# Team766/ros_vision

Measured on NVIDIA B200. Metric: frames/s, higher is better.
Workload: dtype u8

## Files before the change

ros_vision_b200/csrc/kernels_blobs.cu:

```cuda
#include <cuda_runtime.h>
#include <math_constants.h>
#include <stdint.h>

#include <mutex>

#include "dev_types.h"
#include "kernels.h"

namespace b200tag {

static inline unsigned cdivu(unsigned a, unsigned b) { return (a + b - 1) / b; }
__host__ __device__ constexpr uint32_t next_pow2(uint32_t v) { uint32_t r = 1; while (r < v) r <<= 1; return r; }
constexpr uint32_t kMediumCap = 768;
constexpr uint32_t kSortCap = 4096;

__device__ __forceinline__ bool select_blob(const FrameParams &p, uint32_t count, uint32_t minx, uint32_t miny, uint32_t maxx,
                                            uint32_t maxy, int32_t gx, int32_t gy, long long dotsum) {
  if (count < p.min_cluster_pixels) return false;
  if (count > p.max_cluster_pixels) return false;
  if (static_cast<int>((maxx - minx) * (maxy - miny)) < p.min_tag_width) return false;
  const long long a = dotsum * 2 - static_cast<long long>(static_cast<int>(minx + maxx) * gx) -
                      static_cast<long long>(static_cast<int>(miny + maxy) * gy);
  const double d = static_cast<double>(a) * 0.5 - 0.05118 * static_cast<double>(gx) + 0.028581 * static_cast<double>(gy);
  const bool quad_reversed = static_cast<float>(d) < 0.0;
  if (!p.reversed_border && quad_reversed) return false;
  if (!p.normal_border && !quad_reversed) return false;
  return true;
}

template <int MIN_CTAS>
__global__ void __launch_bounds__(256, MIN_CTAS) k_select(FrameParams p) {
  __shared__ uint32_t s_warp[8][6];
  __shared__ unsigned long long s_base;
  __shared__ uint32_t s_pbase, s_mbase, s_lbase, s_hbase;
  const int frame = blockIdx.y;
  const size_t hoff = static_cast<size_t>(frame) * p.hash_cap;
  Counters *ctr = p.counters + frame;
  b200tag_blob *blobs = p.blobs + static_cast<size_t>(frame) * p.blob_cap;
  WorkItem *small_list = p.small_list + static_cast<size_t>(frame) * p.blob_cap;
  WorkItem *large_list = p.large_list + static_cast<size_t>(frame) * p.blob_cap;
  b200tag_blob *clusters = p.clusters ? p.clusters + static_cast<size_t>(frame) * p.cluster_cap : nullptr;
  const int lane = threadIdx.x & 31, warp = threadIdx.x >> 5;
  const uint32_t nocc = min(ctr->num_occupied, p.hash_cap);
  const uint32_t *occupied = p.occupied + hoff;
  const uint32_t nround = (nocc + blockDim.x - 1) / blockDim.x * blockDim.x;
  for (uint32_t oi = blockIdx.x * blockDim.x + threadIdx.x; oi < nround; oi += gridDim.x * blockDim.x) {
    const bool occ = oi < nocc;
    const uint32_t slot = occ ? occupied[oi] : 0u;
    const unsigned long long key = occ ? p.h_key[hoff + slot] : kEmptyKey;
    b200tag_blob rec;
    bool sel = false;
    if (occ) {
      rec.rep0 = static_cast<uint32_t>(key >> 32);
      rec.rep1 = static_cast<uint32_t>(key);
      rec.min_x = 0xffffffffu; rec.min_y = 0xffffffffu; rec.max_x = 0; rec.max_y = 0;
      rec.count = p.h_count[hoff + slot];
      rec.gx_sum = 0; rec.gy_sum = 0; rec.pxgx_plus_pygy_sum = 0;
      rec.slot = slot;
      rec.offset = 0;
      sel = rec.count >= p.min_cluster_pixels && rec.count <= p.max_cluster_pixels;
      rec.selected = 0;
      p.h_key[hoff + slot] = kEmptyKey;
      p.h_count[hoff + slot] = 0;
    }
    const bool small = sel && rec.count <= kSmallBlobPoints;
    const bool medium = sel && !small && rec.count <= kMediumCap;
    const bool huge = sel && rec.count > kSortCap;
    const uint32_t occ_mask = __ballot_sync(0xffffffffu, occ);
    const uint32_t sel_mask = __ballot_sync(0xffffffffu, sel);
    const uint32_t small_mask = __ballot_sync(0xffffffffu, small);
    const uint32_t medium_mask = __ballot_sync(0xffffffffu, medium);
    const uint32_t huge_mask = __ballot_sync(0xffffffffu, huge);
    uint32_t incl = sel ? rec.count : 0u;
#pragma unroll
    for (int o = 1; o < 32; o <<= 1) {
      const uint32_t t = __shfl_up_sync(0xffffffffu, incl, o);
      if (lane >= o) incl += t;
    }
    const uint32_t warp_pts = __shfl_sync(0xffffffffu, incl, 31);
    if (lane == 0) {
      s_warp[warp][0] = __popc(occ_mask);
      s_warp[warp][1] = __popc(sel_mask);
      s_warp[warp][2] = __popc(small_mask);
      s_warp[warp][3] = warp_pts;
      s_warp[warp][4] = __popc(medium_mask);
      s_warp[warp][5] = __popc(huge_mask);
    }
    __syncthreads();
    if (threadIdx.x == 0) {
      uint32_t t0 = 0, t1 = 0, t2 = 0, t3 = 0, t4 = 0, t5 = 0;
      for (int w = 0; w < 8; w++) {
        const uint32_t a0 = s_warp[w][0], a1 = s_warp[w][1], a2 = s_warp[w][2], a3 = s_warp[w][3], a4 = s_warp[w][4], a5 = s_warp[w][5];
        s_warp[w][0] = t0; s_warp[w][1] = t1; s_warp[w][2] = t2; s_warp[w][3] = t3; s_warp[w][4] = t4; s_warp[w][5] = t5;
        t0 += a0; t1 += a1; t2 += a2; t3 += a3; t4 += a4; t5 += a5;
      }
      unsigned long long base = 0;
      uint32_t pb = 0, mb = 0, lb = 0, hb = 0;
      if (t0) {
        const unsigned long long add = (static_cast<unsigned long long>(t0) << 40) | (static_cast<unsigned long long>(t1) << 20) | t2;
        base = atomicAdd(&ctr->alloc, add);
        if (t3) pb = atomicAdd(&ctr->num_seg_points, t3);
        if (t4) mb = atomicAdd(&ctr->num_medium, t4);
        if (t1 - t2 - t4 - t5) lb = atomicAdd(&ctr->num_large, t1 - t2 - t4 - t5);
        if (t5) hb = atomicAdd(&ctr->num_huge, t5);
      }
      s_base = base;
      s_pbase = pb;
      s_mbase = mb;
      s_lbase = lb;
      s_hbase = hb;
    }
    __syncthreads();
    const unsigned long long base = s_base;
    const uint32_t cbase = static_cast<uint32_t>(base >> 40) + s_warp[warp][0];
    const uint32_t bbase = static_cast<uint32_t>(base >> 20) & 0xfffffu;
    const uint32_t sbase = static_cast<uint32_t>(base) & 0xfffffu;
    uint32_t seg_off = 0xffffffffu;
    if (sel) {
      const uint32_t bw = s_warp[warp][1] + __popc(sel_mask & ((1u << lane) - 1u));
      const uint32_t sw = s_warp[warp][2] + __popc(small_mask & ((1u << lane) - 1u));
      const uint32_t mw = s_warp[warp][4] + __popc(medium_mask & ((1u << lane) - 1u));
      const uint32_t hw = s_warp[warp][5] + __popc(huge_mask & ((1u << lane) - 1u));
      const uint32_t cta_pos = medium ? s_mbase + mw
                             : (huge ? p.blob_cap - 1u - (s_hbase + hw) : p.blob_cap - 1u - (s_lbase + (bw - sw - mw - hw)));
      const uint32_t b = bbase + bw;
      const uint32_t off = s_pbase + s_warp[warp][3] + incl - rec.count;
      if (b < p.blob_cap && static_cast<uint64_t>(off) + rec.count <= p.point_cap) {
        rec.offset = off;
        blobs[b] = rec;
        seg_off = off;
        const WorkItem item{b, off, rec.count, 0u};
        if (small) small_list[sbase + sw] = item;
        else if (huge) small_list[cta_pos] = item;
        else large_list[cta_pos] = item;
      } else {
        atomicOr(&ctr->status, B200TAG_ST_BLOBS_OVERFLOW);
        const WorkItem none{0xffffffffu, 0u, 0u, 0u};
        if (small) {
          if (sbase + sw < p.blob_cap) small_list[sbase + sw] = none;
        } else if (cta_pos < p.blob_cap) {
          (huge ? small_list : large_list)[cta_pos] = none;
        }
      }
    }
    if (occ && clusters) {
      const uint32_t c = cbase + __popc(occ_mask & ((1u << lane) - 1u));
      if (c < p.cluster_cap) clusters[c] = rec;
      p.slot_cluster[hoff + slot] = c;
    }
    if (occ) p.slot_off[hoff + slot] = seg_off;
    __syncthreads();
  }
}

template <int U>
__global__ void __launch_bounds__(256) k_scatter(FrameParams p) {
  const int frame = blockIdx.y;
  const Counters *ctr = p.counters + frame;
  const uint32_t np = min(ctr->num_points, p.point_cap);
  const uint64_t *points = p.points + static_cast<size_t>(frame) * p.point_cap;
  const uint32_t *slot_off = p.slot_off + static_cast<size_t>(frame) * p.hash_cap;
  uint32_t *seg = p.seg_pts + static_cast<size_t>(frame) * p.point_cap;
  const uint32_t stride = gridDim.x * blockDim.x;
  for (uint32_t i = blockIdx.x * blockDim.x + threadIdx.x; i < np; i += U * stride) {
    uint64_t pt[U];
    uint32_t off[U];
#pragma unroll
    for (int u = 0; u < U; u++) {
      const uint32_t j = i + u * stride;
      pt[u] = (j < np && j >= i) ? __ldcs(points + j) : ~0ull;
    }
#pragma unroll
    for (int u = 0; u < U; u++) {
      const uint32_t slot = point_slot(pt[u]);
      off[u] = slot < p.hash_cap ? __ldg(slot_off + slot) : 0xffffffffu;
    }
#pragma unroll
    for (int u = 0; u < U; u++)
      if (off[u] != 0xffffffffu) seg[off[u] + point_rank(pt[u])] = point_seg(pt[u]);
  }
}

__global__ void __launch_bounds__(256) k_cluster_extents(FrameParams p) {
  const int frame = blockIdx.y;
  const Counters *ctr = p.counters + frame;
  const uint32_t np = min(ctr->num_points, p.point_cap);
  const uint64_t *points = p.points + static_cast<size_t>(frame) * p.point_cap;
  const uint32_t *slot_cluster = p.slot_cluster + static_cast<size_t>(frame) * p.hash_cap;
  b200tag_blob *clusters = p.clusters + static_cast<size_t>(frame) * p.cluster_cap;
  for (uint32_t i = blockIdx.x * blockDim.x + threadIdx.x; i < np; i += gridDim.x * blockDim.x) {
    const uint64_t pt = points[i];
    const uint32_t slot = point_slot(pt);
    if (slot >= p.hash_cap) continue;
    const uint32_t c = slot_cluster[slot];
    if (c >= p.cluster_cap) continue;
    const uint32_t sp = point_seg(pt);
    const int x = static_cast<int>(sp_x(sp)), y = static_cast<int>(sp_y(sp));
    const int d = static_cast<int>(sp_dir(sp));
    const int gx = sp_b2w(sp) ? dir_dx(d) : -dir_dx(d), gy = sp_b2w(sp) ? dir_dy(d) : -dir_dy(d);
    b200tag_blob *r = clusters + c;
    atomicMin(&r->min_x, static_cast<uint32_t>(x));
    atomicMax(&r->max_x, static_cast<uint32_t>(x));
    atomicMin(&r->min_y, static_cast<uint32_t>(y));
    atomicMax(&r->max_y, static_cast<uint32_t>(y));
    if (gx) atomicAdd(&r->gx_sum, gx);
    if (gy) atomicAdd(&r->gy_sum, gy);
    const int dot = x * gx + y * gy;
    if (dot) atomicAdd(reinterpret_cast<unsigned long long *>(&r->pxgx_plus_pygy_sum), static_cast<unsigned long long>(static_cast<long long>(dot)));
  }
}

__global__ void __launch_bounds__(256) k_cluster_finish(FrameParams p) {
  const int frame = blockIdx.y;
  const Counters *ctr = p.counters + frame;
  const uint32_t nc = min(alloc_clusters(ctr->alloc), p.cluster_cap);
  b200tag_blob *clusters = p.clusters + static_cast<size_t>(frame) * p.cluster_cap;
  for (uint32_t c = blockIdx.x * blockDim.x + threadIdx.x; c < nc; c += gridDim.x * blockDim.x) {
    b200tag_blob *r = clusters + c;
    r->selected = select_blob(p, r->count, r->min_x, r->min_y, r->max_x, r->max_y, r->gx_sum, r->gy_sum, r->pxgx_plus_pygy_sum);
  }
}

constexpr int kLargeThreads = 256;
constexpr int kSmallWarps = 4;

template <int GS>
__device__ __forceinline__ void gsync() {
  if constexpr (GS == 32) __syncwarp();
  else __syncthreads();
}

__device__ __forceinline__ void cmpxchg(unsigned long long *a, uint32_t i, uint32_t l) {
  const unsigned long long x = a[i], y = a[l];
  if (x > y) {
    a[i] = y;
    a[l] = x;
  }
}

template <int GS>
__device__ __noinline__ void bitonic_sort(unsigned long long *a, uint32_t cnt, uint32_t N, uint32_t gt) {
  const uint32_t half = N >> 1;
  for (uint32_t k = 2, lk = 1; k <= N; k <<= 1, lk++) {
    const uint32_t hk = k >> 1;
    for (uint32_t t = gt; t < half; t += GS) {
      const uint32_t blk = t >> (lk - 1), w = t & (hk - 1);
      const uint32_t i = (blk << lk) + w, l = (blk << lk) + k - 1 - w;
      if (l < cnt) cmpxchg(a, i, l);
    }
    if (GS > 32 && (k > 64 || (k == 2 ? false : (k >> 2) >= 64))) __syncthreads();
    else __syncwarp();
    for (uint32_t j = k >> 2; j > 0; j >>= 1) {
      for (uint32_t t = gt; t < half; t += GS) {
        const uint32_t i = ((t & ~(j - 1)) << 1) | (t & (j - 1)), l = i + j;
        if (l < cnt) cmpxchg(a, i, l);
      }
      const bool this_wide = j >= 64;
      const bool next_wide = (j > 1) ? ((j >> 1) >= 64) : ((k << 1) > 64);
      if (GS > 32 && (this_wide || next_wide)) __syncthreads();
      else __syncwarp();
    }
  }
  gsync<GS>();
}

struct Mom {
  long long Mx, My, W, Mxx, Myy, Mxy;
  int N;
};

struct LfStore {
  b200tag_lfp *aos;
  unsigned long long *m64;
  uint32_t *m32;
  uint32_t cap;
};
template <bool AOS>
__device__ __forceinline__ b200tag_lfp lf_load(const LfStore &L, uint32_t i) {
  if constexpr (AOS) return L.aos[i];
  b200tag_lfp r;
  r.Mxx = static_cast<long long>(L.m64[i]);
  r.Myy = static_cast<long long>(L.m64[L.cap + i]);
  r.Mxy = static_cast<long long>(L.m64[2 * L.cap + i]);
  r.Mx = L.m32[i];
  r.My = L.m32[L.cap + i];
  r.W = L.m32[2 * L.cap + i];
  return r;
}
template <bool AOS>
__device__ __forceinline__ void lf_store(const LfStore &L, uint32_t i, const b200tag_lfp &r) {
  if constexpr (AOS) {
    L.aos[i] = r;
    return;
  }
  L.m64[i] = static_cast<unsigned long long>(r.Mxx);
  L.m64[L.cap + i] = static_cast<unsigned long long>(r.Myy);
  L.m64[2 * L.cap + i] = static_cast<unsigned long long>(r.Mxy);
  L.m32[i] = static_cast<uint32_t>(r.Mx);
  L.m32[L.cap + i] = static_cast<uint32_t>(r.My);
  L.m32[2 * L.cap + i] = static_cast<uint32_t>(r.W);
}

template <bool AOS>
__device__ __forceinline__ Mom read_moments(const LfStore &lf, uint32_t cnt, uint32_t i0, uint32_t i1) {
  Mom m;
  if (i0 < i1) {
    m.N = static_cast<int>(i1 - i0 + 1);
    const b200tag_lfp a = lf_load<AOS>(lf, i1);
    m.Mx = a.Mx; m.My = a.My; m.Mxx = a.Mxx; m.Mxy = a.Mxy; m.Myy = a.Myy; m.W = a.W;
    if (i0 > 0) {
      const b200tag_lfp b = lf_load<AOS>(lf, i0 - 1);
      m.Mx -= b.Mx; m.My -= b.My; m.Mxx -= b.Mxx; m.Mxy -= b.Mxy; m.Myy -= b.Myy; m.W -= b.W;
    }
  } else {
    const b200tag_lfp b = lf_load<AOS>(lf, i0 - 1), z = lf_load<AOS>(lf, cnt - 1), a = lf_load<AOS>(lf, i1);
    m.Mx = z.Mx - b.Mx + a.Mx;
    m.My = z.My - b.My + a.My;
    m.Mxx = z.Mxx - b.Mxx + a.Mxx;
    m.Mxy = z.Mxy - b.Mxy + a.Mxy;
    m.Myy = z.Myy - b.Myy + a.Myy;
    m.W = z.W - b.W + a.W;
    m.N = static_cast<int>(cnt - i0 + i1 + 1);
  }
  return m;
}

__device__ __forceinline__ float eig_small_of(const Mom &m, float *hyp_out, long long *Cxx_o, long long *Cxy_o, long long *Cyy_o) {
  const long long Cxx = m.Mxx * m.W - m.Mx * m.Mx;
  const long long Cxy = m.Mxy * m.W - m.Mx * m.My;
  const long long Cyy = m.Myy * m.W - m.My * m.My;
  const float hyp = hypotf(static_cast<float>(Cxx - Cyy), static_cast<float>(2 * Cxy));
  const float eight_w2 = static_cast<float>(static_cast<double>(m.W * m.W) * 8.0);
  const float eig = (static_cast<float>(Cxx + Cyy) - hyp) / eight_w2;
  if (hyp_out) *hyp_out = hyp;
  if (Cxx_o) { *Cxx_o = Cxx; *Cxy_o = Cxy; *Cyy_o = Cyy; }
  return eig;
}

__device__ __forceinline__ void fit_line(const Mom &m, double *lp01, double *lp23, double *err, double *mse) {
  float hyp;
  long long Cxx, Cxy, Cyy;
  const float eig = eig_small_of(m, &hyp, &Cxx, &Cxy, &Cyy);
  if (lp01) {
    lp01[0] = static_cast<double>(static_cast<float>(m.Mx) / static_cast<float>(m.W * 2));
    lp01[1] = static_cast<double>(static_cast<float>(m.My) / static_cast<float>(m.W * 2));
  }
  if (lp23) {
    const float nx1 = static_cast<float>(Cxx - Cyy) - hyp;
    const float ny1 = static_cast<float>(2 * Cxy);
    const float M1 = nx1 * nx1 + ny1 * ny1;
    const float nx2 = static_cast<float>(2 * Cxy);
    const float ny2 = static_cast<float>(Cyy - Cxx) - hyp;
    const float M2 = nx2 * nx2 + ny2 * ny2;
    float nx, ny;
    if (M1 > M2) { nx = nx1; ny = ny1; } else { nx = nx2; ny = ny2; }
    const float len = hypotf(nx, ny);
    lp23[0] = static_cast<double>(nx / len);
    lp23[1] = static_cast<double>(ny / len);
  }
  *err = static_cast<double>(static_cast<float>(m.N) * eig);
  *mse = static_cast<double>(eig);
}

__device__ __forceinline__ int point_weight(const uint8_t *im, int w, int h, int ix, int iy) {
  int W = 1;
  if (ix > 0 && ix + 1 < w && iy > 0 && iy + 1 < h) {
    const int gx = static_cast<int>(__ldg(im + iy * w + ix + 1)) - static_cast<int>(__ldg(im + iy * w + ix - 1));
    const int gy = static_cast<int>(__ldg(im + (iy + 1) * w + ix)) - static_cast<int>(__ldg(im + (iy - 1) * w + ix));
    W = static_cast<int>(__fsqrt_rn(static_cast<float>(gx * gx + gy * gy)) + 1);
  }
  return W;
}

__device__ __forceinline__ uint32_t float_order(float f) {
  const uint32_t u = __float_as_uint(f + 0.0f);
  return (u & 0x80000000u) ? ~u : (u | 0x80000000u);
}

constexpr unsigned long long kNoKey = 0xFFFFFFFFFFFFFFFFull;
constexpr double kDblMax = 1.7976931348623157e308;

template <int WARPS>
struct BlobScratch {
  uint32_t peak_idx[kMaxPeaks];
  uint32_t red_u[WARPS > 1 ? WARPS : 1][4];
  int red_i[WARPS > 1 ? WARPS : 1][3];
  uint32_t npeaks;
  uint32_t nsel;
  uint32_t cur;
};

struct alignas(16) QuadScratch {
  double seg_err[kMaxPeaks][kMaxPeaks];
  double seg_nx[kMaxPeaks][kMaxPeaks], seg_ny[kMaxPeaks][kMaxPeaks];
  double lines[4][4];
  float corners[4][2];
  alignas(16) PeakTable t;
};

__device__ uint8_t d_combos[kNumCombos][4];

__global__ void k_init_combos() {
  int c = 0;
  for (int m0 = 0; m0 < kMaxPeaks - 3; m0++)
    for (int m1 = m0 + 1; m1 < kMaxPeaks - 2; m1++)
      for (int m2 = m1 + 1; m2 < kMaxPeaks - 1; m2++)
        for (int m3 = m2 + 1; m3 < kMaxPeaks; m3++) {
          d_combos[c][0] = m0; d_combos[c][1] = m1; d_combos[c][2] = m2; d_combos[c][3] = m3;
          c++;
        }
}

constexpr int kPeakRegs = 8;

template <int K>
__device__ __forceinline__ unsigned long long top_peaks_regs(const unsigned long long *peaks, uint32_t npk, int lane, uint32_t *nsel_out) {
  static_assert(K == 2 || K == 4 || K == 8, "sorting networks below");
  unsigned long long k[K];
#pragma unroll
  for (int j = 0; j < K; j++) {
    const uint32_t q = static_cast<uint32_t>(lane) + 32u * j;
    k[j] = q < npk ? peaks[q] : kNoKey;
  }
  constexpr int net2[1][2] = {{0, 1}};
  constexpr int net4[5][2] = {{0, 1}, {2, 3}, {0, 2}, {1, 3}, {1, 2}};
  constexpr int net8[19][2] = {{0, 1}, {2, 3}, {4, 5}, {6, 7}, {0, 2}, {1, 3}, {4, 6}, {5, 7}, {1, 2}, {5, 6},
                               {0, 4}, {3, 7}, {1, 5}, {2, 6}, {1, 4}, {3, 6}, {2, 4}, {3, 5}, {3, 4}};
  constexpr int ncmp = K == 2 ? 1 : (K == 4 ? 5 : 19);
#pragma unroll
  for (int c = 0; c < ncmp; c++) {
    const int i0 = K == 2 ? net2[c % 1][0] : (K == 4 ? net4[c % 5][0] : net8[c][0]);
    const int i1 = K == 2 ? net2[c % 1][1] : (K == 4 ? net4[c % 5][1] : net8[c][1]);
    const unsigned long long a = k[i0 % K], b2 = k[i1 % K];
    k[i0 % K] = a < b2 ? a : b2;
    k[i1 % K] = a < b2 ? b2 : a;
  }
  unsigned long long chosen = kNoKey;
  uint32_t nsel = 0;
#pragma unroll 1
  for (int round = 0; round < kMaxPeaks; round++) {
    const uint32_t hi = static_cast<uint32_t>(k[0] >> 32);
    const uint32_t mhi = __reduce_min_sync(0xffffffffu, hi);
    const uint32_t lo = (hi == mhi) ? static_cast<uint32_t>(k[0]) : 0xffffffffu;
    const uint32_t mlo = __reduce_min_sync(0xffffffffu, lo);
    const unsigned long long best = (static_cast<unsigned long long>(mhi) << 32) | mlo;
    if (best == kNoKey) break;
    nsel++;
    if (lane == round) chosen = best;
    if (k[0] == best) {
#pragma unroll
      for (int j = 0; j + 1 < K; j++) k[j] = k[j + 1];
      k[K - 1] = kNoKey;
    }
  }
  *nsel_out = nsel;
  return chosen;
}

__device__ __noinline__ uint32_t top_peaks_many(const unsigned long long *peaks, uint32_t npk, uint32_t *peak_idx, int lane) {
  unsigned long long last = 0;
  uint32_t nsel = 0;
#pragma unroll 1
  for (int round = 0; round < kMaxPeaks; round++) {
    unsigned long long best = kNoKey;
#pragma unroll 1
    for (uint32_t i = lane; i < npk; i += 32) {
      const unsigned long long key = peaks[i];
      if ((round == 0 || key > last) && key < best) best = key;
    }
    {
      const uint32_t hi = static_cast<uint32_t>(best >> 32);
      const uint32_t mhi = __reduce_min_sync(0xffffffffu, hi);
      const uint32_t lo = (hi == mhi) ? static_cast<uint32_t>(best) : 0xffffffffu;
      const uint32_t mlo = __reduce_min_sync(0xffffffffu, lo);
      best = (static_cast<unsigned long long>(mhi) << 32) | mlo;
    }
    if (best == kNoKey) break;
    last = best;
    nsel++;
    if (lane == 0) {
      const uint32_t v2 = static_cast<uint32_t>(best & 0xffffffffu);
      int q = static_cast<int>(nsel) - 2;
      while (q >= 0 && peak_idx[q] > v2) { peak_idx[q + 1] = peak_idx[q]; q--; }
      peak_idx[q + 1] = v2;
    }
    __syncwarp();
  }
  return nsel;
}

struct BlobWork {
  unsigned long long *keys;
  LfStore lf;
  float *errs;
  double *filt;
  unsigned long long *peaks;
  bool keys_in_place;
  uint32_t *hist;
  uint32_t hist_cap;
  uint32_t *tmp;
};

constexpr uint32_t kMaxBucketLoad = 24;

template <int GS, bool AOS, bool KEEP>
__device__ __forceinline__ void fit_one_blob(const FrameParams &p, int frame, Counters *ctr, uint32_t b, uint32_t cnt, uint32_t off,
                                             b200tag_blob *blob_rec, const BlobWork &wk, BlobScratch<GS / 32> &S, long long *scan, uint32_t gt) {
  const size_t n = static_cast<size_t>(p.w) * p.h;
  const uint8_t *quad = p.quad + frame * n;
  const size_t pbase = static_cast<size_t>(frame) * p.point_cap + off;
  const int lane = threadIdx.x & 31;
  const bool first_warp = gt < 32;

  uint32_t *raw = reinterpret_cast<uint32_t *>(wk.errs);
  {
    const uint32_t N = 1u << (32 - __clz(static_cast<int>(cnt - 1)));
    const uint32_t B = min(N, wk.hist_cap);
    for (uint32_t i = gt; i < B; i += GS) wk.hist[i] = 0;
    if (gt == 0) S.npeaks = 0;
    const uint32_t *sp = p.seg_pts + pbase;
    uint32_t mnx = 0xffffffffu, mxx = 0, mny = 0xffffffffu, mxy = 0;
    int sgx = 0, sgy = 0, sdot = 0;
    for (uint32_t i = gt; i < cnt; i += GS) {
      const uint32_t v = __ldcg(sp + i);
      raw[i] = v;
      const uint32_t x = sp_x(v), y = sp_y(v);
      const int d = static_cast<int>(sp_dir(v));
      const int gx = sp_b2w(v) ? dir_dx(d) : -dir_dx(d), gy = sp_b2w(v) ? dir_dy(d) : -dir_dy(d);
      mnx = min(mnx, x); mxx = max(mxx, x); mny = min(mny, y); mxy = max(mxy, y);
      sgx += gx; sgy += gy;
      sdot += static_cast<int>(x) * gx + static_cast<int>(y) * gy;
    }
    mnx = __reduce_min_sync(0xffffffffu, mnx); mxx = __reduce_max_sync(0xffffffffu, mxx);
    mny = __reduce_min_sync(0xffffffffu, mny); mxy = __reduce_max_sync(0xffffffffu, mxy);
    sgx = __reduce_add_sync(0xffffffffu, sgx); sgy = __reduce_add_sync(0xffffffffu, sgy);
    sdot = __reduce_add_sync(0xffffffffu, sdot);
    if constexpr (GS > 32) {
      const int wi = gt >> 5;
      if (lane == 0) {
        S.red_u[wi][0] = mnx; S.red_u[wi][1] = mxx; S.red_u[wi][2] = mny; S.red_u[wi][3] = mxy;
        S.red_i[wi][0] = sgx; S.red_i[wi][1] = sgy; S.red_i[wi][2] = sdot;
      }
      __syncthreads();
      mnx = 0xffffffffu; mxx = 0; mny = 0xffffffffu; mxy = 0; sgx = 0; sgy = 0; sdot = 0;
#pragma unroll
      for (int w = 0; w < GS / 32; w++) {
        mnx = min(mnx, S.red_u[w][0]); mxx = max(mxx, S.red_u[w][1]); mny = min(mny, S.red_u[w][2]); mxy = max(mxy, S.red_u[w][3]);
        sgx += S.red_i[w][0]; sgy += S.red_i[w][1]; sdot += S.red_i[w][2];
      }
    }
    const bool sel = select_blob(p, cnt, mnx, mny, mxx, mxy, sgx, sgy, static_cast<long long>(sdot));
    if (gt == 0) {
      blob_rec->min_x = mnx; blob_rec->min_y = mny; blob_rec->max_x = mxx; blob_rec->max_y = mxy;
      blob_rec->gx_sum = sgx; blob_rec->gy_sum = sgy; blob_rec->pxgx_plus_pygy_sum = sdot;
      blob_rec->selected = sel;
      if (sel) {
        atomicAdd(&ctr->num_selected_blobs, 1u);
        atomicAdd(&ctr->num_selected_points, cnt);
      }
    }
    if (!sel) return;
    if constexpr (GS == 32) __syncwarp();
    const double cx = static_cast<double>(static_cast<float>(static_cast<int>(mnx + mxx)) * 0.5f) + 0.05118;
    const double cy = static_cast<double>(static_cast<float>(static_cast<int>(mny + mxy)) * 0.5f) + -0.028581;

    const uint32_t bk_shift = 26u - (31u - static_cast<uint32_t>(__clz(static_cast<int>(B))));
    uint32_t *th_tmp = wk.tmp, *rk_tmp = wk.tmp + cnt;
#pragma unroll 1
    for (uint32_t i = gt; i < cnt; i += GS) {
      const uint32_t v = raw[i];
      const float fy = static_cast<float>(static_cast<double>(sp_y(v)) - cy);
      const float fx = static_cast<float>(static_cast<double>(sp_x(v)) - cx);
      const float theta = static_cast<float>((static_cast<double>(atan2f(fy, fx)) + 3.14159265358979323846) * 8e6);
      long long ti = llrintf(theta);
      if (ti < 0) ti = 0;
      const uint32_t th = static_cast<uint32_t>(ti & 0xfffffff);
      const uint32_t bk = (th >> bk_shift);
      th_tmp[i] = th;
      rk_tmp[i] = atomicAdd(&wk.hist[bk], 1u);
    }
    gsync<GS>();
    const uint32_t per = B / GS;
    uint32_t sum = 0, mx = 0;
    for (uint32_t j = 0; j < per; j++) {
      const uint32_t c = wk.hist[gt * per + j];
      sum += c;
      mx = max(mx, c);
    }
    uint32_t incl = sum;
#pragma unroll
    for (int o = 1; o < 32; o <<= 1) {
      const uint32_t t = __shfl_up_sync(0xffffffffu, incl, o);
      if (lane >= o) incl += t;
    }
    mx = __reduce_max_sync(0xffffffffu, mx);
    if constexpr (GS > 32) {
      const int wi = gt >> 5;
      if (lane == 31) S.red_u[wi][0] = incl;
      if (lane == 0) S.red_u[wi][1] = mx;
      __syncthreads();
      uint32_t before = 0;
      mx = 0;
#pragma unroll
      for (int w = 0; w < GS / 32; w++) {
        if (w < wi) before += S.red_u[w][0];
        mx = max(mx, S.red_u[w][1]);
      }
      incl += before;
    }
    const bool bucketed = mx <= kMaxBucketLoad && !(p.test_flags & B200TAG_TEST_BITONIC_SORT);
    if (bucketed) {
      uint32_t ex = incl - sum;
      for (uint32_t j = 0; j < per; j++) {
        const uint32_t c = wk.hist[gt * per + j];
        wk.hist[gt * per + j] = ex;
        ex += c;
      }
      gsync<GS>();
      for (uint32_t i = gt; i < cnt; i += GS) {
        const uint32_t v = raw[i], th = th_tmp[i];
        const uint32_t bk = (th >> bk_shift);
        wk.keys[wk.hist[bk] + rk_tmp[i]] = pack_sort_key(th, sp_dir(v), sp_by(v), sp_bx(v));
      }
      gsync<GS>();
      constexpr uint32_t kRankPer = 6;
      if (cnt <= kRankPer * GS) {
        unsigned long long kreg[kRankPer];
        uint32_t preg[kRankPer];
#pragma unroll
        for (uint32_t j = 0; j < kRankPer; j++) {
          const uint32_t q = gt + j * GS;
          kreg[j] = 0;
          preg[j] = 0xffffffffu;
          if (q < cnt) {
            const unsigned long long key = wk.keys[q];
            const uint32_t bk = (key_theta(key) >> bk_shift);
            const uint32_t lo = wk.hist[bk], hi = (bk + 1 < B) ? wk.hist[bk + 1] : cnt;
            uint32_t pos = lo;
#pragma unroll 1
            for (uint32_t i = lo; i < hi; i++) pos += wk.keys[i] < key;
            kreg[j] = key;
            preg[j] = pos;
          }
        }
        gsync<GS>();
#pragma unroll
        for (uint32_t j = 0; j < kRankPer; j++)
          if (preg[j] != 0xffffffffu) wk.keys[preg[j]] = kreg[j];
      } else {
        for (uint32_t j = 0; j < per; j++) {
          const uint32_t bk = gt * per + j;
          const uint32_t lo = wk.hist[bk], hi = (bk + 1 < B) ? wk.hist[bk + 1] : cnt;
          for (uint32_t i = lo + 1; i < hi; i++) {
            const unsigned long long key = wk.keys[i];
            uint32_t q = i;
            while (q > lo && wk.keys[q - 1] > key) {
              wk.keys[q] = wk.keys[q - 1];
              q--;
            }
            wk.keys[q] = key;
          }
        }
      }
      gsync<GS>();
    } else {
      for (uint32_t i = gt; i < cnt; i += GS) {
        const uint32_t v = raw[i];
        wk.keys[i] = pack_sort_key(th_tmp[i], sp_dir(v), sp_by(v), sp_bx(v));
      }
      gsync<GS>();
      bitonic_sort<GS>(wk.keys, cnt, N, gt);
    }
  }
  if (KEEP && !wk.keys_in_place) {
    uint64_t *out = p.seg_keys + pbase;
#pragma unroll 1
    for (uint32_t i = gt; i < cnt; i += GS) out[i] = wk.keys[i];
  }

  int *wbuf = reinterpret_cast<int *>(wk.errs);
  if constexpr (!AOS) {
    {
      const int wi = static_cast<int>(gt >> 5);
      const uint32_t L = ((cnt + GS - 1) / GS) | 1u;
      const uint32_t c_lo = min(cnt, gt * L), c_hi = min(cnt, c_lo + L);
      unsigned long long t_Mxx = 0, t_Myy = 0, t_Mxy = 0;
      uint32_t t_Mx = 0, t_My = 0, t_W = 0;
  #pragma unroll 2
      for (uint32_t i = c_lo; i < c_hi; i++) {
        const unsigned long long k = wk.keys[i];
        const uint32_t d = key_dir(k);
        const uint32_t ix2 = 2 * key_bx(k) + dir_dx(d) + 1, iy2 = 2 * key_by(k) + dir_dy(d) + 1;
        const uint32_t W = static_cast<uint32_t>(point_weight(quad, p.w, p.h, static_cast<int>(ix2 / 2), static_cast<int>(iy2 / 2)));
        wbuf[i] = static_cast<int>(W);
        const uint32_t wx = W * ix2, wy = W * iy2;
        t_Mx += wx; t_My += wy; t_W += W;
        t_Mxx += static_cast<unsigned long long>(wx) * ix2;
        t_Mxy += static_cast<unsigned long long>(wx) * iy2;
        t_Myy += static_cast<unsigned long long>(wy) * iy2;
      }
      unsigned long long s_Mxx = t_Mxx, s_Myy = t_Myy, s_Mxy = t_Mxy, s_Mx = t_Mx, s_My = t_My, s_W = t_W;
  #pragma unroll
      for (int o = 1; o < 32; o <<= 1) {
        const unsigned long long u_Mxx = __shfl_up_sync(0xffffffffu, s_Mxx, o), u_Myy = __shfl_up_sync(0xffffffffu, s_Myy, o);
        const unsigned long long u_Mxy = __shfl_up_sync(0xffffffffu, s_Mxy, o);
        const uint32_t u_Mx = __shfl_up_sync(0xffffffffu, static_cast<uint32_t>(s_Mx), o), u_My = __shfl_up_sync(0xffffffffu, static_cast<uint32_t>(s_My), o);
        const uint32_t u_W = __shfl_up_sync(0xffffffffu, static_cast<uint32_t>(s_W), o);
        if (lane >= o) { s_Mx += u_Mx; s_My += u_My; s_W += u_W; s_Mxx += u_Mxx; s_Myy += u_Myy; s_Mxy += u_Mxy; }
      }
      unsigned long long c_Mxx = s_Mxx - t_Mxx, c_Myy = s_Myy - t_Myy, c_Mxy = s_Mxy - t_Mxy;
      unsigned long long c_Mx = s_Mx - t_Mx, c_My = s_My - t_My, c_W = s_W - t_W;
      if constexpr (GS > 32) {
        unsigned long long *tot = reinterpret_cast<unsigned long long *>(scan);
        if (lane == 31) {
          tot[wi * 6 + 0] = s_Mxx; tot[wi * 6 + 1] = s_Myy; tot[wi * 6 + 2] = s_Mxy;
          tot[wi * 6 + 3] = s_Mx;  tot[wi * 6 + 4] = s_My;  tot[wi * 6 + 5] = s_W;
        }
        __syncthreads();
        for (int w = 0; w < wi; w++) {
          c_Mxx += tot[w * 6 + 0]; c_Myy += tot[w * 6 + 1]; c_Mxy += tot[w * 6 + 2];
          c_Mx += tot[w * 6 + 3];  c_My += tot[w * 6 + 4];  c_W += tot[w * 6 + 5];
        }
      }
  #pragma unroll 2
      for (uint32_t i = c_lo; i < c_hi; i++) {
        const unsigned long long k = wk.keys[i];
        const uint32_t d = key_dir(k);
        const uint32_t ix2 = 2 * key_bx(k) + dir_dx(d) + 1, iy2 = 2 * key_by(k) + dir_dy(d) + 1;
        const uint32_t W = static_cast<uint32_t>(wbuf[i]);
        const uint32_t wx = W * ix2, wy = W * iy2;
        c_Mx += wx; c_My += wy; c_W += W;
        c_Mxx += static_cast<unsigned long long>(wx) * ix2;
        c_Mxy += static_cast<unsigned long long>(wx) * iy2;
        c_Myy += static_cast<unsigned long long>(wy) * iy2;
        b200tag_lfp o;
        o.Mxx = static_cast<long long>(c_Mxx); o.Myy = static_cast<long long>(c_Myy); o.Mxy = static_cast<long long>(c_Mxy);
        o.Mx = static_cast<long long>(c_Mx); o.My = static_cast<long long>(c_My); o.W = static_cast<long long>(c_W);
        lf_store<AOS>(wk.lf, i, o);
      }
    }
  } else {
  #pragma unroll 2
    for (uint32_t i = gt; i < cnt; i += GS) {
      const unsigned long long k = wk.keys[i];
      const uint32_t d = key_dir(k);
      const int ix2 = static_cast<int>(2 * key_bx(k)) + dir_dx(d) + 1, iy2 = static_cast<int>(2 * key_by(k)) + dir_dy(d) + 1;
      wbuf[i] = point_weight(quad, p.w, p.h, ix2 / 2, iy2 / 2);
    }
    gsync<GS>();
    {
      constexpr int kWarps = GS / 32;
      const int wi = static_cast<int>(gt >> 5);
      const uint32_t per_warp = ((cnt + kWarps - 1) / kWarps + 31u) & ~31u;
      const uint32_t w_lo = min(cnt, wi * per_warp), w_hi = min(cnt, w_lo + per_warp);
      unsigned long long c_Mxx = 0, c_Myy = 0, c_Mxy = 0, c_Mx = 0, c_My = 0, c_W = 0;
      if constexpr (GS > 32) {
        unsigned long long t_Mxx = 0, t_Myy = 0, t_Mxy = 0;
        uint32_t t_Mx = 0, t_My = 0, t_W = 0;
        for (uint32_t i = w_lo + lane; i < w_hi; i += 32) {
          const unsigned long long k = wk.keys[i];
          const uint32_t d = key_dir(k);
          const uint32_t ix2 = 2 * key_bx(k) + dir_dx(d) + 1, iy2 = 2 * key_by(k) + dir_dy(d) + 1;
          const uint32_t W = static_cast<uint32_t>(wbuf[i]);
          const uint32_t wx = W * ix2, wy = W * iy2;
          t_Mx += wx; t_My += wy; t_W += W;
          t_Mxx += static_cast<unsigned long long>(wx) * ix2;
          t_Mxy += static_cast<unsigned long long>(wx) * iy2;
          t_Myy += static_cast<unsigned long long>(wy) * iy2;
        }
        unsigned long long r_Mx = t_Mx, r_My = t_My, r_W = t_W;
  #pragma unroll
        for (int o = 16; o > 0; o >>= 1) {
          t_Mxx += __shfl_xor_sync(0xffffffffu, t_Mxx, o);
          t_Myy += __shfl_xor_sync(0xffffffffu, t_Myy, o);
          t_Mxy += __shfl_xor_sync(0xffffffffu, t_Mxy, o);
          r_Mx += __shfl_xor_sync(0xffffffffu, r_Mx, o);
          r_My += __shfl_xor_sync(0xffffffffu, r_My, o);
          r_W += __shfl_xor_sync(0xffffffffu, r_W, o);
        }
        unsigned long long *tot = reinterpret_cast<unsigned long long *>(scan);
        if (lane == 0) {
          tot[wi * 6 + 0] = t_Mxx; tot[wi * 6 + 1] = t_Myy; tot[wi * 6 + 2] = t_Mxy;
          tot[wi * 6 + 3] = r_Mx;  tot[wi * 6 + 4] = r_My;  tot[wi * 6 + 5] = r_W;
        }
        __syncthreads();
        for (int w = 0; w < wi; w++) {
          c_Mxx += tot[w * 6 + 0]; c_Myy += tot[w * 6 + 1]; c_Mxy += tot[w * 6 + 2];
          c_Mx += tot[w * 6 + 3];  c_My += tot[w * 6 + 4];  c_W += tot[w * 6 + 5];
        }
      }
  #pragma unroll 1
      for (uint32_t base = w_lo; base < w_hi; base += 32) {
        const uint32_t i = base + lane;
        uint32_t s_Mx = 0, s_My = 0, s_W = 0;
        unsigned long long s_Mxx = 0, s_Myy = 0, s_Mxy = 0;
        if (i < w_hi) {
          const unsigned long long k = wk.keys[i];
          const uint32_t d = key_dir(k);
          const uint32_t ix2 = 2 * key_bx(k) + dir_dx(d) + 1, iy2 = 2 * key_by(k) + dir_dy(d) + 1;
          const uint32_t W = static_cast<uint32_t>(wbuf[i]);
          const uint32_t wx = W * ix2, wy = W * iy2;
          s_Mx = wx; s_My = wy; s_W = W;
          s_Mxx = static_cast<unsigned long long>(wx) * ix2;
          s_Mxy = static_cast<unsigned long long>(wx) * iy2;
          s_Myy = static_cast<unsigned long long>(wy) * iy2;
        }
  #pragma unroll
        for (int o = 1; o < 32; o <<= 1) {
          const uint32_t u_Mx = __shfl_up_sync(0xffffffffu, s_Mx, o), u_My = __shfl_up_sync(0xffffffffu, s_My, o);
          const uint32_t u_W = __shfl_up_sync(0xffffffffu, s_W, o);
          const unsigned long long u_Mxx = __shfl_up_sync(0xffffffffu, s_Mxx, o), u_Myy = __shfl_up_sync(0xffffffffu, s_Myy, o);
          const unsigned long long u_Mxy = __shfl_up_sync(0xffffffffu, s_Mxy, o);
          if (lane >= o) { s_Mx += u_Mx; s_My += u_My; s_W += u_W; s_Mxx += u_Mxx; s_Myy += u_Myy; s_Mxy += u_Mxy; }
        }
        if (i < w_hi) {
          b200tag_lfp o;
          o.Mxx = static_cast<long long>(c_Mxx + s_Mxx); o.Myy = static_cast<long long>(c_Myy + s_Myy);
          o.Mxy = static_cast<long long>(c_Mxy + s_Mxy);
          o.Mx = static_cast<long long>(c_Mx + s_Mx); o.My = static_cast<long long>(c_My + s_My); o.W = static_cast<long long>(c_W + s_W);
          lf_store<AOS>(wk.lf, i, o);
        }
        c_Mxx += __shfl_sync(0xffffffffu, s_Mxx, 31); c_Myy += __shfl_sync(0xffffffffu, s_Myy, 31);
        c_Mxy += __shfl_sync(0xffffffffu, s_Mxy, 31);
        c_Mx += __shfl_sync(0xffffffffu, s_Mx, 31); c_My += __shfl_sync(0xffffffffu, s_My, 31); c_W += __shfl_sync(0xffffffffu, s_W, 31);
      }
    }
  }
  gsync<GS>();
  if (KEEP && !AOS) {
    b200tag_lfp *out = p.lfp + pbase;
#pragma unroll 1
    for (uint32_t i = gt; i < cnt; i += GS) out[i] = lf_load<AOS>(wk.lf, i);
  }

  const uint32_t ksz = min(20u, cnt / 12u);
#pragma unroll 1
  for (uint32_t i = gt; i < cnt; i += GS) {
    uint32_t i0 = i + cnt - ksz, i1 = i + ksz;
    if (i0 >= cnt) i0 -= cnt;
    if (i1 >= cnt) i1 -= cnt;
    const Mom m = read_moments<AOS>(wk.lf, cnt, i0, i1);
    const float eig = eig_small_of(m, nullptr, nullptr, nullptr, nullptr);
    wk.errs[i] = static_cast<float>(m.N) * eig;
  }
  gsync<GS>();
  if (KEEP && wk.errs != p.errs + pbase) {
    float *out = p.errs + pbase;
#pragma unroll 1
    for (uint32_t i = gt; i < cnt; i += GS) out[i] = wk.errs[i];
  }
#pragma unroll 1
  for (uint32_t i = gt; i < cnt; i += GS) {
    const float kf[7] = {0.01110899634659290314f, 0.13533528149127960205f, 0.60653066635131835938f, 1.0f,
                         0.60653066635131835938f, 0.13533528149127960205f, 0.01110899634659290314f};
    double acc = 0.0;
    uint32_t q = i + cnt - 3;
    if (q >= cnt) q -= cnt;
#pragma unroll
    for (int j = 0; j < 7; j++) {
      const double e = static_cast<double>(wk.errs[q]);
      acc += e * static_cast<double>(kf[j]);
      if (++q == cnt) q = 0;
    }
    wk.filt[i] = acc;
  }
  gsync<GS>();
  if (KEEP && wk.filt != p.filt + pbase) {
    double *out = p.filt + pbase;
#pragma unroll 1
    for (uint32_t i = gt; i < cnt; i += GS) out[i] = wk.filt[i];
  }

#pragma unroll 1
  for (uint32_t i = gt; i < cnt; i += GS) {
    const double m = wk.filt[i];
    const double bv = wk.filt[i == 0 ? cnt - 1 : i - 1], av = wk.filt[i + 1 == cnt ? 0 : i + 1];
    if (m > bv && m > av) {
      const uint32_t at = atomicAdd(&S.npeaks, 1u);
      wk.peaks[at] = (static_cast<unsigned long long>(float_order(static_cast<float>(-m))) << 32) | i;
    }
  }
  gsync<GS>();
  const uint32_t npk = S.npeaks;
  if (npk == 0) return;

  uint32_t fq_slot = 0;
  if (first_warp) {
    if (lane == 0) fq_slot = atomicAdd(&ctr->num_fit_quads, 1u);
    uint32_t nsel = 0;
    if (npk <= 32) {
      unsigned long long v = lane < static_cast<int>(npk) ? wk.peaks[lane] : kNoKey;
#pragma unroll
      for (int k = 2; k <= 32; k <<= 1) {
#pragma unroll
        for (int j = k >> 1; j > 0; j >>= 1) {
          const unsigned long long other = __shfl_xor_sync(0xffffffffu, v, j);
          const bool take_min = ((lane & k) == 0) == ((lane & j) == 0);
          v = (take_min == (other < v)) ? other : v;
        }
      }
      nsel = min(npk, static_cast<uint32_t>(kMaxPeaks));
      const uint32_t my_idx = static_cast<uint32_t>(v & 0xffffffffu);
      uint32_t rank = 0;
#pragma unroll
      for (int m = 0; m < kMaxPeaks; m++) {
        const uint32_t o = __shfl_sync(0xffffffffu, my_idx, m);
        rank += (m < static_cast<int>(nsel)) && (o < my_idx);
      }
      if (lane < static_cast<int>(nsel)) S.peak_idx[rank] = my_idx;
    } else if (npk <= 32 * kPeakRegs) {
      const unsigned long long chosen = npk <= 64    ? top_peaks_regs<2>(wk.peaks, npk, lane, &nsel)
                                        : npk <= 128 ? top_peaks_regs<4>(wk.peaks, npk, lane, &nsel)
                                                     : top_peaks_regs<8>(wk.peaks, npk, lane, &nsel);
      const uint32_t my_idx = static_cast<uint32_t>(chosen & 0xffffffffu);
      uint32_t rank = 0;
#pragma unroll
      for (int m = 0; m < kMaxPeaks; m++) {
        const uint32_t o = __shfl_sync(0xffffffffu, my_idx, m);
        rank += (m < static_cast<int>(nsel)) && (o < my_idx);
      }
      if (lane < static_cast<int>(nsel)) S.peak_idx[rank] = my_idx;
    } else {
      nsel = top_peaks_many(wk.peaks, npk, S.peak_idx, lane);
    }
    if (lane == 0) S.nsel = nsel;
    __syncwarp();
  }

  if (first_warp) {
    const uint32_t nm = S.nsel;
    const uint32_t fq = __shfl_sync(0xffffffffu, fq_slot, 0);
    if (fq < p.blob_cap) {
      PeakTable *t = p.peak_tables + static_cast<size_t>(frame) * p.blob_cap + fq;
      if (lane == 0) {
        t->blob = b; t->cnt = cnt; t->nsel = nm; t->npk = npk; t->rep0 = blob_rec->rep0; t->rep1 = blob_rec->rep1;
        t->last = lf_load<AOS>(wk.lf, cnt - 1);
      }
      if (lane < static_cast<int>(nm)) {
        const uint32_t i = S.peak_idx[lane];
        t->idx[lane] = i;
        t->at[lane] = lf_load<AOS>(wk.lf, i);
        b200tag_lfp z;
        z.Mxx = 0; z.Myy = 0; z.Mxy = 0; z.Mx = 0; z.My = 0; z.W = 0;
        t->before[lane] = i > 0 ? lf_load<AOS>(wk.lf, i - 1) : z;
      }
    }
  }
}

__device__ __forceinline__ Mom table_moments(const PeakTable &T, int a, int c) {
  const uint32_t i0 = T.idx[a], i1 = T.idx[c];
  const b200tag_lfp hi = T.at[c], lo = T.before[a];
  Mom m;
  if (i0 < i1) {
    m.N = static_cast<int>(i1 - i0 + 1);
    m.Mx = hi.Mx; m.My = hi.My; m.Mxx = hi.Mxx; m.Mxy = hi.Mxy; m.Myy = hi.Myy; m.W = hi.W;
    if (i0 > 0) { m.Mx -= lo.Mx; m.My -= lo.My; m.Mxx -= lo.Mxx; m.Mxy -= lo.Mxy; m.Myy -= lo.Myy; m.W -= lo.W; }
  } else {
    const b200tag_lfp z = T.last;
    m.Mx = z.Mx - lo.Mx + hi.Mx;
    m.My = z.My - lo.My + hi.My;
    m.Mxx = z.Mxx - lo.Mxx + hi.Mxx;
    m.Mxy = z.Mxy - lo.Mxy + hi.Mxy;
    m.Myy = z.Myy - lo.Myy + hi.Myy;
    m.W = z.W - lo.W + hi.W;
    m.N = static_cast<int>(T.cnt - i0 + i1 + 1);
  }
  return m;
}

constexpr int kQuadWarps = 4;

__global__ void __launch_bounds__(kQuadWarps * 32, 8) k_quads(FrameParams p) {
  __shared__ QuadScratch s_q[kQuadWarps];
  const int frame = blockIdx.y;
  const int lane = threadIdx.x & 31;
  QuadScratch &S = s_q[threadIdx.x >> 5];
  Counters *ctr = p.counters + frame;
  const uint32_t nfq = min(ctr->num_fit_quads, p.blob_cap);
  const PeakTable *tables = p.peak_tables + static_cast<size_t>(frame) * p.blob_cap;
  for (uint32_t fq = blockIdx.x * kQuadWarps + (threadIdx.x >> 5); fq < nfq; fq += gridDim.x * kQuadWarps) {
    __syncwarp();
    {
      constexpr uint32_t kPieces = sizeof(PeakTable) / 16, kPer = (kPieces + 31) / 32;
      const uint4 *src = reinterpret_cast<const uint4 *>(tables + fq);
      uint4 *dst = reinterpret_cast<uint4 *>(&S.t);
      uint4 v[kPer];
#pragma unroll
      for (uint32_t k = 0; k < kPer; k++)
        if (lane + 32 * k < kPieces) v[k] = __ldcg(src + lane + 32 * k);
#pragma unroll
      for (uint32_t k = 0; k < kPer; k++)
        if (lane + 32 * k < kPieces) dst[lane + 32 * k] = v[k];
    }
    __syncwarp();
    const PeakTable &T = S.t;
    const uint32_t b = T.blob, cnt = T.cnt, npk = T.npk;

  const int nm = static_cast<int>(T.nsel);
  const double max_mse = static_cast<double>(p.max_line_fit_mse);
  const uint32_t inv_nm1 = nm > 1 ? 65535u / static_cast<uint32_t>(nm - 1) + 1u : 0u;
  for (int t = lane; t < nm * (nm - 1); t += 32) {
    const int a = static_cast<int>((static_cast<uint32_t>(t) * inv_nm1) >> 16);
    int c = t - a * (nm - 1);
    c += c >= a;
    const Mom mo = table_moments(T, a, c);
    double err, mse, nrm[2] = {0.0, 0.0};
    fit_line(mo, nullptr, a < c ? nrm : nullptr, &err, &mse);
    S.seg_err[a][c] = (mse > max_mse) ? kDblMax : err;
    S.seg_nx[a][c] = nrm[0];
    S.seg_ny[a][c] = nrm[1];
  }
  __syncwarp();

  {
    const double max_dot = static_cast<double>(p.cos_critical_rad);
    double my_err = kDblMax;
    int my_rank = kNumCombos;
    for (int c = lane; c < kNumCombos; c += 32) {
      const uchar4 cm = *reinterpret_cast<const uchar4 *>(d_combos[c]);
      const int m0 = cm.x, m1 = cm.y, m2 = cm.z, m3 = cm.w;
      if (m3 >= nm) continue;
      const double e01 = S.seg_err[m0][m1];
      if (e01 == kDblMax) continue;
      const double e12 = S.seg_err[m1][m2];
      if (e12 == kDblMax) continue;
      const double dot = S.seg_nx[m0][m1] * S.seg_nx[m1][m2] + S.seg_ny[m0][m1] * S.seg_ny[m1][m2];
      if (fabs(dot) > max_dot) continue;
      const double e23 = S.seg_err[m2][m3];
      if (e23 == kDblMax) continue;
      const double e30 = S.seg_err[m3][m0];
      if (e30 == kDblMax) continue;
      const double tot = e01 + e12 + e23 + e30;
      if (tot < my_err) { my_err = tot; my_rank = c; }
    }
#pragma unroll
    for (int o = 16; o > 0; o >>= 1) {
      const double oe = __shfl_xor_sync(0xffffffffu, my_err, o);
      const int orank = __shfl_xor_sync(0xffffffffu, my_rank, o);
      if (oe < my_err || (oe == my_err && orank < my_rank)) { my_err = oe; my_rank = orank; }
    }

    const double best = my_err;
    const int bi = my_rank < kNumCombos ? my_rank : 0;
    const bool valid = best < static_cast<double>(p.max_line_fit_mse * static_cast<float>(cnt));
    b200tag_fit_quad *fqo = (fq < p.blob_cap) ? (p.fit_quads + static_cast<size_t>(frame) * p.blob_cap + fq) : nullptr;
    if (lane == 0 && fqo) {
      fqo->blob_index = b;
      fqo->valid = valid;
      fqo->num_peaks = static_cast<int32_t>(npk);
      fqo->err = best;
    }
    if (lane < 4) {
      uint32_t i0 = 0;
      Mom mo;
      if (valid) {
        i0 = T.idx[d_combos[bi][lane]];
        mo = table_moments(T, d_combos[bi][lane], d_combos[bi][(lane + 1) & 3]);
        double err, mse;
        fit_line(mo, S.lines[lane], S.lines[lane] + 2, &err, &mse);
      }
      if (fqo) {
        fqo->indices[lane] = i0;
        b200tag_moments mm = b200tag_moments{0, 0, 0, 0, 0, 0, 0, 0};
        if (valid) { mm.Mx = mo.Mx; mm.My = mo.My; mm.W = mo.W; mm.Mxx = mo.Mxx; mm.Myy = mo.Myy; mm.Mxy = mo.Mxy; mm.N = mo.N; }
        fqo->moments[lane] = mm;
      }
    }
    __syncwarp();
    if (valid) {
      bool bad = false;
      if (lane < 4) {
        const int i = lane, nx = (lane + 1) & 3;
        const double A00 = S.lines[i][3], A01 = -S.lines[nx][3];
        const double A10 = -S.lines[i][2], A11 = S.lines[nx][2];
        const double B0 = -S.lines[i][0] + S.lines[nx][0];
        const double B1 = -S.lines[i][1] + S.lines[nx][1];
        const double det = A00 * A11 - A10 * A01;
        const double W00 = A11 / det, W01 = -A01 / det;
        if (fabs(det) < 0.001) bad = true;
        const double L0 = W00 * B0 + W01 * B1;
        S.corners[i][0] = static_cast<float>(S.lines[i][0] + L0 * A00);
        S.corners[i][1] = static_cast<float>(S.lines[i][1] + L0 * A10);
      }
      bad = __any_sync(0xffffffffu, bad);
      __syncwarp();
      float elen = 0;
      if (lane < 6) {
        const int a = (0x032210 >> (4 * lane)) & 0xf, c = (0x203021 >> (4 * lane)) & 0xf;
        elen = hypotf(S.corners[c][0] - S.corners[a][0], S.corners[c][1] - S.corners[a][1]);
      }
      float elens[6];
#pragma unroll
      for (int i = 0; i < 6; i++) elens[i] = __shfl_sync(0xffffffffu, elen, i);
      if (lane == 0 && !bad) {
        float cr[4][2];
        for (int j = 0; j < 4; j++) { cr[j][0] = S.corners[j][0]; cr[j][1] = S.corners[j][1]; }
        {
          float area = 0;
          float pp;
          pp = (elens[0] + elens[1] + elens[2]) / 2;
          area += sqrtf(pp * (pp - elens[0]) * (pp - elens[1]) * (pp - elens[2]));
          pp = (elens[3] + elens[4] + elens[5]) / 2;
          area += sqrtf(pp * (pp - elens[3]) * (pp - elens[4]) * (pp - elens[5]));
          if (static_cast<double>(area) < 0.95 * p.min_tag_width * p.min_tag_width) bad = true;
        }
        if (!bad) {
          for (int i = 0; i < 4; i++) {
            const int i0 = i, i1 = (i + 1) & 3, i2 = (i + 2) & 3;
            const float dx1 = cr[i1][0] - cr[i0][0], dy1 = cr[i1][1] - cr[i0][1];
            const float dx2 = cr[i2][0] - cr[i1][0], dy2 = cr[i2][1] - cr[i1][1];
            const float cos_dtheta = (dx1 * dx2 + dy1 * dy2) / sqrtf((dx1 * dx1 + dy1 * dy1) * (dx2 * dx2 + dy2 * dy2));
            if (fabsf(cos_dtheta) > p.cos_critical_rad || dx1 * dy2 < dy1 * dx2) { bad = true; break; }
          }
        }
        if (!bad) {
          const float f = static_cast<float>(p.f);
          if (f > 1) {
            for (int j = 0; j < 4; j++) {
              cr[j][0] = (cr[j][0] - 0.5f) * f + 0.5f;
              cr[j][1] = (cr[j][1] - 0.5f) * f + 0.5f;
            }
          }
          const uint32_t qi = atomicAdd(&ctr->num_quads, 1u);
          if (qi < p.quad_cap) {
            b200tag_quad &q = (p.quads + static_cast<size_t>(frame) * p.quad_cap)[qi];
            for (int j = 0; j < 4; j++) { q.corners[j][0] = cr[j][0]; q.corners[j][1] = cr[j][1]; }
            q.reversed_border = p.reversed_border && !p.normal_border;
            q.blob_index = b;
            q.rep0 = T.rep0;
            q.rep1 = T.rep1;
          } else {
            atomicOr(&ctr->status, B200TAG_ST_QUADS_OVERFLOW);
          }
        }
      }
    }
  }
  }
}

struct SmallWarpShared {
  unsigned long long keys[kSmallBlobPoints];
  unsigned long long lf64[3 * kSmallBlobPoints];
  uint32_t lf32[3 * kSmallBlobPoints];
  alignas(16) float errs[kSmallBlobPoints];
  BlobScratch<1> scratch;
};

template <bool KEEP>
__global__ void __launch_bounds__(kSmallWarps * 32, 6) k_fit_small(FrameParams p) {
  extern __shared__ __align__(16) unsigned char smem_raw[];
  SmallWarpShared &S = reinterpret_cast<SmallWarpShared *>(smem_raw)[threadIdx.x >> 5];
  const int frame = blockIdx.y;
  const int lane = threadIdx.x & 31;
  Counters *ctr = p.counters + frame;
  b200tag_blob *blobs = p.blobs + static_cast<size_t>(frame) * p.blob_cap;
  const WorkItem *list = p.small_list + static_cast<size_t>(frame) * p.blob_cap;
  const uint32_t nlist = min(alloc_small(ctr->alloc), p.blob_cap);
  BlobWork wk;
  wk.keys = S.keys;
  wk.lf.aos = nullptr; wk.lf.m64 = S.lf64; wk.lf.m32 = S.lf32; wk.lf.cap = kSmallBlobPoints;
  wk.errs = S.errs;
  wk.filt = reinterpret_cast<double *>(S.keys);
  wk.peaks = reinterpret_cast<unsigned long long *>(S.errs);
  wk.keys_in_place = false;
  wk.hist = reinterpret_cast<uint32_t *>(S.lf64);
  wk.hist_cap = next_pow2(kSmallBlobPoints);
  wk.tmp = wk.hist + next_pow2(kSmallBlobPoints);
  uint32_t nxt = 0;
  if (lane == 0) nxt = atomicAdd(&ctr->next_small, 1u);
  while (true) {
    __syncwarp();
    const uint32_t li = __shfl_sync(0xffffffffu, nxt, 0);
    if (li >= nlist) break;
    if (lane == 0) nxt = atomicAdd(&ctr->next_small, 1u);
    const WorkItem item = list[li];
    const uint32_t b = item.blob, off = item.offset, cnt = item.count;
    if (b >= p.blob_cap) continue;
    if (cnt > kSmallBlobPoints) continue;
    fit_one_blob<32, false, KEEP>(p, frame, ctr, b, cnt, off, blobs + b, wk, S.scratch, nullptr, lane);
  }
}

template <int THREADS, uint32_t KEY_CAP, uint32_t LF_CAP>
struct CtaShared {
  static constexpr bool kHasB = KEY_CAP > LF_CAP;
  static constexpr uint32_t kScanWords = kHasB ? (KEY_CAP / 2 > 6 * THREADS ? KEY_CAP / 2 : 6 * THREADS) : 0;
  static constexpr size_t kBytesA = static_cast<size_t>(LF_CAP) * 48;
  static constexpr size_t kBytesB = kHasB ? static_cast<size_t>(KEY_CAP) * 12 + static_cast<size_t>(kScanWords) * 8 : 0;
  alignas(16) unsigned char buf[kBytesA > kBytesB ? kBytesA : kBytesB];
  long long tot[6 * (THREADS / 32)];
  BlobScratch<THREADS / 32> scratch;

  __device__ unsigned long long *a_keys() { return reinterpret_cast<unsigned long long *>(buf); }
  __device__ unsigned long long *a_lf64() { return reinterpret_cast<unsigned long long *>(buf) + LF_CAP; }
  __device__ uint32_t *a_lf32() { return reinterpret_cast<uint32_t *>(buf + static_cast<size_t>(LF_CAP) * 32); }
  __device__ float *a_errs() { return reinterpret_cast<float *>(buf + static_cast<size_t>(LF_CAP) * 44); }
  __device__ unsigned long long *b_keys() { return reinterpret_cast<unsigned long long *>(buf); }
  __device__ float *b_errs() { return reinterpret_cast<float *>(buf + static_cast<size_t>(KEY_CAP) * 8); }
  __device__ long long *b_scan() { return reinterpret_cast<long long *>(buf + static_cast<size_t>(KEY_CAP) * 12); }
};
static_assert(kMediumCap % 4 == 0 && kSortCap % 4 == 0, "16-byte alignment of the carved arrays");

template <int THREADS, uint32_t KEY_CAP, uint32_t LF_CAP, uint32_t MIN_CNT, uint32_t MAX_CNT, int MIN_CTAS, bool KEEP>
__global__ void __launch_bounds__(THREADS, MIN_CTAS) k_fit_cta(FrameParams p, int tier) {
  using Shared = CtaShared<THREADS, KEY_CAP, LF_CAP>;
  extern __shared__ __align__(16) unsigned char smem_raw[];
  Shared &S = *reinterpret_cast<Shared *>(smem_raw);
  const int frame = blockIdx.y;
  const int tid = threadIdx.x;
  Counters *ctr = p.counters + frame;
  b200tag_blob *blobs = p.blobs + static_cast<size_t>(frame) * p.blob_cap;
  const WorkItem *list = (tier == 2 ? p.small_list : p.large_list) + static_cast<size_t>(frame) * p.blob_cap;
  const uint32_t nlist = min(tier == 0 ? ctr->num_medium : (tier == 1 ? ctr->num_large : ctr->num_huge), p.blob_cap);
  constexpr uint32_t kScanHist = (KEY_CAP / 2 > 6 * THREADS) ? KEY_CAP : ((6u * THREADS * 2u >= 2048u) ? 2048u : 1024u);
  uint32_t *next = tier == 0 ? &ctr->next_medium : (tier == 1 ? &ctr->next_large : &ctr->next_huge);
  uint32_t nxt = 0;
  if (tid == 0) nxt = atomicAdd(next, 1u);
  while (true) {
    __syncthreads();
    if (tid == 0) S.scratch.cur = nxt;
    __syncthreads();
    const uint32_t li = S.scratch.cur;
    if (li >= nlist) break;
    if (tid == 0) nxt = atomicAdd(next, 1u);
    const WorkItem item = list[tier == 0 ? li : p.blob_cap - 1u - li];
    const uint32_t b = item.blob, blob_off = item.offset, blob_cnt = item.count;
    if (b >= p.blob_cap) continue;
    if (blob_cnt < MIN_CNT || blob_cnt > MAX_CNT) continue;
    const size_t pbase = static_cast<size_t>(frame) * p.point_cap + blob_off;
    BlobWork wk;
    constexpr bool kHasSmemLf = LF_CAP > 0;
    constexpr bool kHasGlobalLf = MAX_CNT > LF_CAP;
    constexpr bool kHasInPlace = MAX_CNT > KEY_CAP;
    const bool lf32_ok = LF_CAP <= 1452 || !kHasGlobalLf ||
                         static_cast<uint64_t>(blob_cnt) * 361u * (2u * static_cast<uint32_t>(max(p.w, p.h)) + 1u) < (1ull << 32);
    if (kHasSmemLf && blob_cnt <= LF_CAP && lf32_ok) {
      wk.keys = S.a_keys(); wk.errs = S.a_errs();
      wk.lf.aos = nullptr; wk.lf.m64 = S.a_lf64(); wk.lf.m32 = S.a_lf32(); wk.lf.cap = LF_CAP;
      wk.filt = reinterpret_cast<double *>(S.a_keys());
      wk.peaks = reinterpret_cast<unsigned long long *>(S.a_errs());
      wk.keys_in_place = false;
      wk.hist = reinterpret_cast<uint32_t *>(S.a_lf64()); wk.hist_cap = next_pow2(LF_CAP > 0 ? LF_CAP : 1); wk.tmp = wk.hist + next_pow2(LF_CAP > 0 ? LF_CAP : 1);
      fit_one_blob<THREADS, false, KEEP>(p, frame, ctr, b, blob_cnt, blob_off, blobs + b, wk, S.scratch, S.tot, tid);
    } else if (kHasGlobalLf && KEY_CAP > LF_CAP && blob_cnt <= KEY_CAP) {
      wk.keys = S.b_keys(); wk.errs = S.b_errs();
      wk.lf.aos = p.lfp + pbase; wk.lf.m64 = nullptr; wk.lf.m32 = nullptr; wk.lf.cap = 0;
      wk.filt = reinterpret_cast<double *>(S.b_keys());
      wk.peaks = reinterpret_cast<unsigned long long *>(S.b_errs());
      wk.keys_in_place = false;
      wk.hist = reinterpret_cast<uint32_t *>(S.b_scan()); wk.hist_cap = kScanHist; wk.tmp = reinterpret_cast<uint32_t *>(p.lfp + pbase);
      fit_one_blob<THREADS, true, KEEP>(p, frame, ctr, b, blob_cnt, blob_off, blobs + b, wk, S.scratch, S.b_scan(), tid);
    } else if (kHasInPlace) {
      wk.keys = reinterpret_cast<unsigned long long *>(p.seg_keys + pbase);
      wk.lf.aos = p.lfp + pbase; wk.lf.m64 = nullptr; wk.lf.m32 = nullptr; wk.lf.cap = 0;
      wk.errs = p.errs + pbase; wk.filt = p.filt + pbase;
      wk.peaks = reinterpret_cast<unsigned long long *>(p.peak_ws + static_cast<size_t>(frame) * (p.point_cap / 2 + 1) + blob_off / 2);
      wk.keys_in_place = true;
      wk.hist = reinterpret_cast<uint32_t *>(S.b_scan()); wk.hist_cap = kScanHist; wk.tmp = reinterpret_cast<uint32_t *>(p.lfp + pbase);
      fit_one_blob<THREADS, true, KEEP>(p, frame, ctr, b, blob_cnt, blob_off, blobs + b, wk, S.scratch, S.b_scan(), tid);
    }
  }
}

using MediumShared = CtaShared<128, kMediumCap, kMediumCap>;
constexpr uint32_t kLargeLfCap = 1536;
using LargeShared = CtaShared<kLargeThreads, kSortCap, kLargeLfCap>;
static_assert(sizeof(LargeShared) <= 76800 - 1024, "three CTAs of the large tier per SM");
static_assert(sizeof(MediumShared) <= 37888, "shared memory of the medium tier");
#define K_FIT_MEDIUM(KEEP) k_fit_cta<128, kMediumCap, kMediumCap, kSmallBlobPoints + 1, kMediumCap, 6, KEEP>
#define K_FIT_LARGE(KEEP) k_fit_cta<kLargeThreads, kSortCap, kLargeLfCap, kMediumCap + 1, kSortCap, 3, KEEP>
constexpr int kHugeThreads = 512;
constexpr uint32_t kHugeCap = 8192;
using HugeShared = CtaShared<kHugeThreads, kHugeCap, 0>;
#define K_FIT_HUGE(KEEP) k_fit_cta<kHugeThreads, kHugeCap, 0, kSortCap + 1, 0xffffffffu, (KEEP) ? 1 : 2, KEEP>
using Large512Shared = CtaShared<kHugeThreads, kSortCap, kSortCap>;
#define K_FIT_LARGE512(KEEP) k_fit_cta<kHugeThreads, kSortCap, kSortCap, kMediumCap + 1, kSortCap, 1, KEEP>
static_assert(sizeof(Large512Shared) <= 227 * 1024, "shared memory of the low-latency large tier");
constexpr int kLowLatencyFrames = 4;

void launch_blobs_init(cudaStream_t s) {
  static bool dev_ready[64] = {false};
  static std::mutex mu;
  std::lock_guard<std::mutex> lock(mu);
  int dev = 0;
  cudaGetDevice(&dev);
  if (dev >= 0 && dev < 64 && !dev_ready[dev]) {
    cudaFuncSetAttribute(k_fit_small<false>, cudaFuncAttributeMaxDynamicSharedMemorySize, static_cast<int>(sizeof(SmallWarpShared) * kSmallWarps));
    cudaFuncSetAttribute(k_fit_small<true>, cudaFuncAttributeMaxDynamicSharedMemorySize, static_cast<int>(sizeof(SmallWarpShared) * kSmallWarps));
    cudaFuncSetAttribute(K_FIT_MEDIUM(false), cudaFuncAttributeMaxDynamicSharedMemorySize, static_cast<int>(sizeof(MediumShared)));
    cudaFuncSetAttribute(K_FIT_MEDIUM(true), cudaFuncAttributeMaxDynamicSharedMemorySize, static_cast<int>(sizeof(MediumShared)));
    cudaFuncSetAttribute(K_FIT_LARGE(false), cudaFuncAttributeMaxDynamicSharedMemorySize, static_cast<int>(sizeof(LargeShared)));
    cudaFuncSetAttribute(K_FIT_LARGE(true), cudaFuncAttributeMaxDynamicSharedMemorySize, static_cast<int>(sizeof(LargeShared)));
    cudaFuncSetAttribute(K_FIT_HUGE(false), cudaFuncAttributeMaxDynamicSharedMemorySize, static_cast<int>(sizeof(HugeShared)));
    cudaFuncSetAttribute(K_FIT_HUGE(true), cudaFuncAttributeMaxDynamicSharedMemorySize, static_cast<int>(sizeof(HugeShared)));
    cudaFuncSetAttribute(K_FIT_LARGE512(false), cudaFuncAttributeMaxDynamicSharedMemorySize, static_cast<int>(sizeof(Large512Shared)));
    cudaFuncSetAttribute(K_FIT_LARGE512(true), cudaFuncAttributeMaxDynamicSharedMemorySize, static_cast<int>(sizeof(Large512Shared)));
    k_init_combos<<<1, 1, 0, s>>>();
    dev_ready[dev] = true;
  }
}

int launch_blobs(const FrameParams &p, int frames, cudaStream_t s, KernelTimer *kt, const SideStreams *side) {
  if (kt) kt->begin("select", s);
  if (exp_flags() & 64) k_select<1><<<dim3(max(1u, min(16u, cdivu(148u * 4u, frames))), frames), 256, 0, s>>>(p);
  else k_select<8><<<dim3(max(1u, min(16u, 148u * 8u / static_cast<unsigned>(frames))), frames), 256, 0, s>>>(p);
  if (kt) kt->end(s);
  if (kt) kt->begin("scatter", s);
  if (exp_flags() & 1) k_scatter<1><<<dim3(max(8u, min(592u, cdivu(4736u, frames))), frames), 256, 0, s>>>(p);
  else if (exp_flags() & 32) k_scatter<8><<<dim3(max(8u, min(592u, cdivu(4736u, frames))), frames), 256, 0, s>>>(p);
  else k_scatter<4><<<dim3(max(8u, min(592u, cdivu(4736u, frames))), frames), 256, 0, s>>>(p);
  if (kt) kt->end(s);
  int launches = 6;
  if (p.clusters) {
    k_cluster_extents<<<dim3(max(8u, min(592u, cdivu(4736u, frames))), frames), 256, 0, s>>>(p);
    k_cluster_finish<<<dim3(16, frames), 256, 0, s>>>(p);
    launches += 2;
  }
  const bool fork = side && side->s[0] && side->s[1] && side->s[2];
  cudaStream_t s_large = fork ? side->s[0] : s, s_medium = fork ? side->s[1] : s, s_huge = fork ? side->s[2] : s;
  if (fork) {
    cudaEventRecord(side->fork, s);
    cudaStreamWaitEvent(s_large, side->fork, 0);
    cudaStreamWaitEvent(s_medium, side->fork, 0);
    cudaStreamWaitEvent(s_huge, side->fork, 0);
  }
  if (kt) kt->begin("fit_huge", s);
  {
    const dim3 g(max(1u, min(148u, cdivu(592u, frames))), frames);
    if (p.keep_stages) K_FIT_HUGE(true)<<<g, kHugeThreads, sizeof(HugeShared), s_huge>>>(p, 2);
    else K_FIT_HUGE(false)<<<g, kHugeThreads, sizeof(HugeShared), s_huge>>>(p, 2);
  }
  if (kt) kt->end(s);
  if (kt) kt->begin("fit_large", s);
  const bool lf32_ok = static_cast<uint64_t>(kSortCap) * 361u * (2u * static_cast<uint32_t>(max(p.w, p.h)) + 1u) < (1ull << 32);
  if (frames <= kLowLatencyFrames && lf32_ok) {
    const dim3 g(max(1u, min(148u, cdivu(592u, frames))), frames);
    if (p.keep_stages) K_FIT_LARGE512(true)<<<g, kHugeThreads, sizeof(Large512Shared), s_large>>>(p, 1);
    else K_FIT_LARGE512(false)<<<g, kHugeThreads, sizeof(Large512Shared), s_large>>>(p, 1);
  } else {
    const dim3 g(max(3u, min(444u, cdivu(1776u, frames))), frames);
    if (p.keep_stages) K_FIT_LARGE(true)<<<g, kLargeThreads, sizeof(LargeShared), s_large>>>(p, 1);
    else K_FIT_LARGE(false)<<<g, kLargeThreads, sizeof(LargeShared), s_large>>>(p, 1);
  }
  if (kt) kt->end(s);
  if (kt) kt->begin("fit_medium", s);
  {
    const dim3 g(max(4u, min(740u, cdivu(2960u, frames))), frames);
    if (p.keep_stages) K_FIT_MEDIUM(true)<<<g, 128, sizeof(MediumShared), s_medium>>>(p, 0);
    else K_FIT_MEDIUM(false)<<<g, 128, sizeof(MediumShared), s_medium>>>(p, 0);
  }
  if (kt) kt->end(s);
  if (kt) kt->begin("fit_small", s);
  {
    const dim3 g(max(4u, min(740u, cdivu(2960u, frames))), frames);
    if (p.keep_stages) k_fit_small<true><<<g, kSmallWarps * 32, sizeof(SmallWarpShared) * kSmallWarps, s>>>(p);
    else k_fit_small<false><<<g, kSmallWarps * 32, sizeof(SmallWarpShared) * kSmallWarps, s>>>(p);
  }
  if (kt) kt->end(s);
  if (fork) {
    cudaEventRecord(side->join[0], s_large);
    cudaEventRecord(side->join[1], s_medium);
    cudaEventRecord(side->join[2], s_huge);
    cudaStreamWaitEvent(s, side->join[0], 0);
    cudaStreamWaitEvent(s, side->join[1], 0);
    cudaStreamWaitEvent(s, side->join[2], 0);
  }
  if (kt) kt->begin("quads", s);
  k_quads<<<dim3(max(2u, min(592u, cdivu(2368u, frames))), frames), kQuadWarps * 32, 0, s>>>(p);
  if (kt) kt->end(s);
  return launches + 1;
}

}
```

Baseline: 58650.

## Replace per-point line-fit prefix arrays with per-thread moment sums and sliding windows

Adds a new line-fit mode for large blobs. Each thread keeps a prefix sum of six moments over its contiguous chunk, with the point weight packed into the sort key, instead of materialising a full per-point prefix array. The error window and the Gaussian filter are then computed with per-thread sliding windows, and angle and rank are packed into one temp word. The goal is to keep mid-to-large blobs in shared memory instead of global memory and cut memory traffic. In exchange there is more recomputation at window edges, new tier caps, and fewer CTAs per SM for the KEEP large tier.

```diff
diff --git a/ros_vision_b200/csrc/kernels_blobs.cu b/ros_vision_b200/csrc/kernels_blobs.cu
--- a/ros_vision_b200/csrc/kernels_blobs.cu
+++ b/ros_vision_b200/csrc/kernels_blobs.cu
@@ -269,51 +269,96 @@
   int N;
 };
 
-struct LfStore {
-  b200tag_lfp *aos;
-  unsigned long long *m64;
-  uint32_t *m32;
-  uint32_t cap;
+struct M6 {
+  unsigned long long Mxx, Myy, Mxy, Mx, My, W;
 };
-template <bool AOS>
-__device__ __forceinline__ b200tag_lfp lf_load(const LfStore &L, uint32_t i) {
-  if constexpr (AOS) return L.aos[i];
+__device__ __forceinline__ M6 m6_zero() { return M6{0, 0, 0, 0, 0, 0}; }
+__device__ __forceinline__ void m6_add(M6 &a, const M6 &b) {
+  a.Mxx += b.Mxx; a.Myy += b.Myy; a.Mxy += b.Mxy; a.Mx += b.Mx; a.My += b.My; a.W += b.W;
+}
+__device__ __forceinline__ void m6_sub(M6 &a, const M6 &b) {
+  a.Mxx -= b.Mxx; a.Myy -= b.Myy; a.Mxy -= b.Mxy; a.Mx -= b.Mx; a.My -= b.My; a.W -= b.W;
+}
+__device__ __forceinline__ b200tag_lfp m6_lfp(const M6 &a) {
   b200tag_lfp r;
-  r.Mxx = static_cast<long long>(L.m64[i]);
-  r.Myy = static_cast<long long>(L.m64[L.cap + i]);
-  r.Mxy = static_cast<long long>(L.m64[2 * L.cap + i]);
-  r.Mx = L.m32[i];
-  r.My = L.m32[L.cap + i];
-  r.W = L.m32[2 * L.cap + i];
+  r.Mxx = static_cast<long long>(a.Mxx); r.Myy = static_cast<long long>(a.Myy); r.Mxy = static_cast<long long>(a.Mxy);
+  r.Mx = static_cast<long long>(a.Mx); r.My = static_cast<long long>(a.My); r.W = static_cast<long long>(a.W);
   return r;
 }
-template <bool AOS>
-__device__ __forceinline__ void lf_store(const LfStore &L, uint32_t i, const b200tag_lfp &r) {
-  if constexpr (AOS) {
-    L.aos[i] = r;
-    return;
-  }
-  L.m64[i] = static_cast<unsigned long long>(r.Mxx);
-  L.m64[L.cap + i] = static_cast<unsigned long long>(r.Myy);
-  L.m64[2 * L.cap + i] = static_cast<unsigned long long>(r.Mxy);
-  L.m32[i] = static_cast<uint32_t>(r.Mx);
-  L.m32[L.cap + i] = static_cast<uint32_t>(r.My);
-  L.m32[2 * L.cap + i] = static_cast<uint32_t>(r.W);
-}
-
-template <bool AOS>
-__device__ __forceinline__ Mom read_moments(const LfStore &lf, uint32_t cnt, uint32_t i0, uint32_t i1) {
+
+constexpr int kKeyWeightShift = 54;
+__device__ __forceinline__ uint32_t key_weight(unsigned long long k) { return static_cast<uint32_t>(k >> kKeyWeightShift) & 0x1ffu; }
+__device__ __forceinline__ void m6_add_point(M6 &s, unsigned long long k, uint32_t W) {
+  const uint32_t d = key_dir(k);
+  const uint32_t ix2 = 2 * key_bx(k) + dir_dx(d) + 1, iy2 = 2 * key_by(k) + dir_dy(d) + 1;
+  const uint32_t wx = W * ix2, wy = W * iy2;
+  s.Mx += wx; s.My += wy; s.W += W;
+  s.Mxx += static_cast<unsigned long long>(wx) * ix2;
+  s.Mxy += static_cast<unsigned long long>(wx) * iy2;
+  s.Myy += static_cast<unsigned long long>(wy) * iy2;
+}
+__device__ __forceinline__ M6 m6_point(unsigned long long k) {
+  M6 s = m6_zero();
+  m6_add_point(s, k, key_weight(k));
+  return s;
+}
+
+template <int GS>
+__device__ __forceinline__ M6 sums_at(const unsigned long long *sums, uint32_t t) {
+  return M6{sums[t], sums[GS + t], sums[2 * GS + t], sums[3 * GS + t], sums[4 * GS + t], sums[5 * GS + t]};
+}
+template <int GS>
+__device__ __forceinline__ M6 prefix_at(const unsigned long long *keys, const unsigned long long *sums, uint32_t L, uint32_t cnt,
+                                        uint32_t j) {
+  const uint32_t o = j / L, lo = o * L, hi = min(cnt, lo + L);
+  M6 s;
+  if (2 * (j - lo) < hi - lo) {
+    s = o ? sums_at<GS>(sums, o - 1) : m6_zero();
+#pragma unroll 4
+    for (uint32_t q = lo; q <= j; q++) m6_add(s, m6_point(keys[q]));
+  } else {
+    s = sums_at<GS>(sums, o);
+#pragma unroll 4
+    for (uint32_t q = j + 1; q < hi; q++) m6_sub(s, m6_point(keys[q]));
+  }
+  return s;
+}
+template <int GS>
+__device__ __forceinline__ M6 cyclic_prefix_at(const unsigned long long *keys, const unsigned long long *sums, uint32_t L, uint32_t cnt, int j) {
+  if (j == -1) return m6_zero();
+  const M6 total = sums_at<GS>(sums, GS - 1);
+  if (j < 0) {
+    M6 s = prefix_at<GS>(keys, sums, L, cnt, static_cast<uint32_t>(j + static_cast<int>(cnt)));
+    m6_sub(s, total);
+    return s;
+  }
+  if (j >= static_cast<int>(cnt)) {
+    M6 s = prefix_at<GS>(keys, sums, L, cnt, static_cast<uint32_t>(j - static_cast<int>(cnt)));
+    m6_add(s, total);
+    return s;
+  }
+  return prefix_at<GS>(keys, sums, L, cnt, static_cast<uint32_t>(j));
+}
+
+struct BlobWork;
+template <int MODE>
+__device__ __forceinline__ b200tag_lfp lf_load(const BlobWork &wk, uint32_t i);
+template <int MODE>
+__device__ __forceinline__ void lf_store(const BlobWork &wk, uint32_t i, const b200tag_lfp &r);
+
+template <int MODE>
+__device__ __forceinline__ Mom read_moments(const BlobWork &lf, uint32_t cnt, uint32_t i0, uint32_t i1) {
   Mom m;
   if (i0 < i1) {
     m.N = static_cast<int>(i1 - i0 + 1);
-    const b200tag_lfp a = lf_load<AOS>(lf, i1);
+    const b200tag_lfp a = lf_load<MODE>(lf, i1);
     m.Mx = a.Mx; m.My = a.My; m.Mxx = a.Mxx; m.Mxy = a.Mxy; m.Myy = a.Myy; m.W = a.W;
     if (i0 > 0) {
-      const b200tag_lfp b = lf_load<AOS>(lf, i0 - 1);
+      const b200tag_lfp b = lf_load<MODE>(lf, i0 - 1);
       m.Mx -= b.Mx; m.My -= b.My; m.Mxx -= b.Mxx; m.Mxy -= b.Mxy; m.Myy -= b.Myy; m.W -= b.W;
     }
   } else {
-    const b200tag_lfp b = lf_load<AOS>(lf, i0 - 1), z = lf_load<AOS>(lf, cnt - 1), a = lf_load<AOS>(lf, i1);
+    const b200tag_lfp b = lf_load<MODE>(lf, i0 - 1), z = lf_load<MODE>(lf, cnt - 1), a = lf_load<MODE>(lf, i1);
     m.Mx = z.Mx - b.Mx + a.Mx;
     m.My = z.My - b.My + a.My;
     m.Mxx = z.Mxx - b.Mxx + a.Mxx;
@@ -489,9 +534,14 @@
   return nsel;
 }
 
+constexpr int kLfGlobal = 0, kLfArrays = 1, kLfThreadSums = 2;
 struct BlobWork {
   unsigned long long *keys;
-  LfStore lf;
+  b200tag_lfp *lf;
+  unsigned long long *m64;
+  uint32_t *m32;
+  uint32_t lf_cap;
+  unsigned long long *sums;
   float *errs;
   double *filt;
   unsigned long long *peaks;
@@ -501,9 +551,35 @@
   uint32_t *tmp;
 };
 
+template <int MODE>
+__device__ __forceinline__ b200tag_lfp lf_load(const BlobWork &wk, uint32_t i) {
+  if constexpr (MODE == kLfGlobal) return wk.lf[i];
+  b200tag_lfp r;
+  r.Mxx = static_cast<long long>(wk.m64[i]);
+  r.Myy = static_cast<long long>(wk.m64[wk.lf_cap + i]);
+  r.Mxy = static_cast<long long>(wk.m64[2 * wk.lf_cap + i]);
+  r.Mx = wk.m32[i];
+  r.My = wk.m32[wk.lf_cap + i];
+  r.W = wk.m32[2 * wk.lf_cap + i];
+  return r;
+}
+template <int MODE>
+__device__ __forceinline__ void lf_store(const BlobWork &wk, uint32_t i, const b200tag_lfp &r) {
+  if constexpr (MODE == kLfGlobal) {
+    wk.lf[i] = r;
+    return;
+  }
+  wk.m64[i] = static_cast<unsigned long long>(r.Mxx);
+  wk.m64[wk.lf_cap + i] = static_cast<unsigned long long>(r.Myy);
+  wk.m64[2 * wk.lf_cap + i] = static_cast<unsigned long long>(r.Mxy);
+  wk.m32[i] = static_cast<uint32_t>(r.Mx);
+  wk.m32[wk.lf_cap + i] = static_cast<uint32_t>(r.My);
+  wk.m32[2 * wk.lf_cap + i] = static_cast<uint32_t>(r.W);
+}
+
 constexpr uint32_t kMaxBucketLoad = 24;
 
-template <int GS, bool AOS, bool KEEP>
+template <int GS, int MODE, bool KEEP>
 __device__ __forceinline__ void fit_one_blob(const FrameParams &p, int frame, Counters *ctr, uint32_t b, uint32_t cnt, uint32_t off,
                                              b200tag_blob *blob_rec, const BlobWork &wk, BlobScratch<GS / 32> &S, long long *scan, uint32_t gt) {
   const size_t n = static_cast<size_t>(p.w) * p.h;
@@ -565,7 +641,6 @@
     const double cy = static_cast<double>(static_cast<float>(static_cast<int>(mny + mxy)) * 0.5f) + -0.028581;
 
     const uint32_t bk_shift = 26u - (31u - static_cast<uint32_t>(__clz(static_cast<int>(B))));
-    uint32_t *th_tmp = wk.tmp, *rk_tmp = wk.tmp + cnt;
 #pragma unroll 1
     for (uint32_t i = gt; i < cnt; i += GS) {
       const uint32_t v = raw[i];
@@ -576,8 +651,7 @@
       if (ti < 0) ti = 0;
       const uint32_t th = static_cast<uint32_t>(ti & 0xfffffff);
       const uint32_t bk = (th >> bk_shift);
-      th_tmp[i] = th;
-      rk_tmp[i] = atomicAdd(&wk.hist[bk], 1u);
+      wk.tmp[i] = (th << 6) | min(atomicAdd(&wk.hist[bk], 1u), 63u);
     }
     gsync<GS>();
     const uint32_t per = B / GS;
@@ -618,9 +692,9 @@
       }
       gsync<GS>();
       for (uint32_t i = gt; i < cnt; i += GS) {
-        const uint32_t v = raw[i], th = th_tmp[i];
+        const uint32_t v = raw[i], th = wk.tmp[i] >> 6;
         const uint32_t bk = (th >> bk_shift);
-        wk.keys[wk.hist[bk] + rk_tmp[i]] = pack_sort_key(th, sp_dir(v), sp_by(v), sp_bx(v));
+        wk.keys[wk.hist[bk] + (wk.tmp[i] & 63u)] = pack_sort_key(th, sp_dir(v), sp_by(v), sp_bx(v));
       }
       gsync<GS>();
       constexpr uint32_t kRankPer = 6;
@@ -666,7 +740,7 @@
     } else {
       for (uint32_t i = gt; i < cnt; i += GS) {
         const uint32_t v = raw[i];
-        wk.keys[i] = pack_sort_key(th_tmp[i], sp_dir(v), sp_by(v), sp_bx(v));
+        wk.keys[i] = pack_sort_key(wk.tmp[i] >> 6, sp_dir(v), sp_by(v), sp_bx(v));
       }
       gsync<GS>();
       bitonic_sort<GS>(wk.keys, cnt, N, gt);
@@ -676,14 +750,58 @@
     uint64_t *out = p.seg_keys + pbase;
 #pragma unroll 1
     for (uint32_t i = gt; i < cnt; i += GS) out[i] = wk.keys[i];
-  }
-
-  int *wbuf = reinterpret_cast<int *>(wk.errs);
-  if constexpr (!AOS) {
+    if constexpr (MODE == kLfThreadSums) gsync<GS>();
+  }
+
+  const uint32_t L = ((cnt + GS - 1) / GS) | 1u;
+  const uint32_t c_lo = min(cnt, gt * L), c_hi = min(cnt, c_lo + L);
+  if constexpr (MODE == kLfThreadSums) {
+    const int wi = static_cast<int>(gt >> 5);
+    M6 t = m6_zero();
+#pragma unroll 2
+    for (uint32_t i = c_lo; i < c_hi; i++) {
+      const unsigned long long k = wk.keys[i];
+      const uint32_t d = key_dir(k);
+      const uint32_t ix2 = 2 * key_bx(k) + dir_dx(d) + 1, iy2 = 2 * key_by(k) + dir_dy(d) + 1;
+      const uint32_t W = static_cast<uint32_t>(point_weight(quad, p.w, p.h, static_cast<int>(ix2 / 2), static_cast<int>(iy2 / 2)));
+      const unsigned long long kw = k | (static_cast<unsigned long long>(W) << kKeyWeightShift);
+      wk.keys[i] = kw;
+      m6_add_point(t, kw, W);
+    }
+    M6 s = t;
+#pragma unroll
+    for (int o = 1; o < 32; o <<= 1) {
+      M6 u;
+      u.Mxx = __shfl_up_sync(0xffffffffu, s.Mxx, o); u.Myy = __shfl_up_sync(0xffffffffu, s.Myy, o);
+      u.Mxy = __shfl_up_sync(0xffffffffu, s.Mxy, o); u.Mx = __shfl_up_sync(0xffffffffu, s.Mx, o);
+      u.My = __shfl_up_sync(0xffffffffu, s.My, o);   u.W = __shfl_up_sync(0xffffffffu, s.W, o);
+      if (lane >= o) m6_add(s, u);
+    }
+    if constexpr (GS > 32) {
+      unsigned long long *tot = reinterpret_cast<unsigned long long *>(scan);
+      if (lane == 31) {
+        tot[wi * 6 + 0] = s.Mxx; tot[wi * 6 + 1] = s.Myy; tot[wi * 6 + 2] = s.Mxy;
+        tot[wi * 6 + 3] = s.Mx;  tot[wi * 6 + 4] = s.My;  tot[wi * 6 + 5] = s.W;
+      }
+      __syncthreads();
+      for (int w = 0; w < wi; w++) m6_add(s, M6{tot[w * 6 + 0], tot[w * 6 + 1], tot[w * 6 + 2], tot[w * 6 + 3], tot[w * 6 + 4], tot[w * 6 + 5]});
+    }
+    wk.sums[gt] = s.Mxx; wk.sums[GS + gt] = s.Myy; wk.sums[2 * GS + gt] = s.Mxy;
+    wk.sums[3 * GS + gt] = s.Mx; wk.sums[4 * GS + gt] = s.My; wk.sums[5 * GS + gt] = s.W;
+    if constexpr (KEEP) {
+      m6_sub(s, t);
+      b200tag_lfp *out = p.lfp + pbase;
+#pragma unroll 1
+      for (uint32_t i = c_lo; i < c_hi; i++) {
+        const unsigned long long k = wk.keys[i];
+        m6_add_point(s, k, key_weight(k));
+        out[i] = m6_lfp(s);
+      }
+    }
+  } else if constexpr (MODE == kLfArrays) {
+    int *wbuf = reinterpret_cast<int *>(wk.errs);
     {
       const int wi = static_cast<int>(gt >> 5);
-      const uint32_t L = ((cnt + GS - 1) / GS) | 1u;
-      const uint32_t c_lo = min(cnt, gt * L), c_hi = min(cnt, c_lo + L);
       unsigned long long t_Mxx = 0, t_Myy = 0, t_Mxy = 0;
       uint32_t t_Mx = 0, t_My = 0, t_W = 0;
   #pragma unroll 2
@@ -736,10 +854,11 @@
         b200tag_lfp o;
         o.Mxx = static_cast<long long>(c_Mxx); o.Myy = static_cast<long long>(c_Myy); o.Mxy = static_cast<long long>(c_Mxy);
         o.Mx = static_cast<long long>(c_Mx); o.My = static_cast<long long>(c_My); o.W = static_cast<long long>(c_W);
-        lf_store<AOS>(wk.lf, i, o);
+        lf_store<MODE>(wk, i, o);
       }
     }
   } else {
+    int *wbuf = reinterpret_cast<int *>(wk.errs);
   #pragma unroll 2
     for (uint32_t i = gt; i < cnt; i += GS) {
       const unsigned long long k = wk.keys[i];
@@ -818,7 +937,7 @@
           o.Mxx = static_cast<long long>(c_Mxx + s_Mxx); o.Myy = static_cast<long long>(c_Myy + s_Myy);
           o.Mxy = static_cast<long long>(c_Mxy + s_Mxy);
           o.Mx = static_cast<long long>(c_Mx + s_Mx); o.My = static_cast<long long>(c_My + s_My); o.W = static_cast<long long>(c_W + s_W);
-          lf_store<AOS>(wk.lf, i, o);
+          lf_store<MODE>(wk, i, o);
         }
         c_Mxx += __shfl_sync(0xffffffffu, s_Mxx, 31); c_Myy += __shfl_sync(0xffffffffu, s_Myy, 31);
         c_Mxy += __shfl_sync(0xffffffffu, s_Mxy, 31);
@@ -827,21 +946,47 @@
     }
   }
   gsync<GS>();
-  if (KEEP && !AOS) {
+  if (KEEP && MODE == kLfArrays) {
     b200tag_lfp *out = p.lfp + pbase;
 #pragma unroll 1
-    for (uint32_t i = gt; i < cnt; i += GS) out[i] = lf_load<AOS>(wk.lf, i);
+    for (uint32_t i = gt; i < cnt; i += GS) out[i] = lf_load<MODE>(wk, i);
   }
 
   const uint32_t ksz = min(20u, cnt / 12u);
+  if constexpr (MODE == kLfThreadSums) {
+    if (c_lo < c_hi) {
+      M6 win = gt ? sums_at<GS>(wk.sums, gt - 1) : m6_zero();
+      m6_add(win, m6_point(wk.keys[c_lo]));
+      m6_sub(win, cyclic_prefix_at<GS>(wk.keys, wk.sums, L, cnt, static_cast<int>(c_lo) - 2 * static_cast<int>(ksz) - 1));
+      const int N = static_cast<int>(2 * ksz + 1);
+      uint32_t o = c_lo + cnt - ksz, tr = c_lo + cnt - 2 * ksz - 1;
+      if (o >= cnt) o -= cnt;
+      if (tr >= cnt) tr -= cnt;
 #pragma unroll 1
-  for (uint32_t i = gt; i < cnt; i += GS) {
-    uint32_t i0 = i + cnt - ksz, i1 = i + ksz;
-    if (i0 >= cnt) i0 -= cnt;
-    if (i1 >= cnt) i1 -= cnt;
-    const Mom m = read_moments<AOS>(wk.lf, cnt, i0, i1);
-    const float eig = eig_small_of(m, nullptr, nullptr, nullptr, nullptr);
-    wk.errs[i] = static_cast<float>(m.N) * eig;
+      for (uint32_t j = c_lo;;) {
+        Mom m;
+        m.Mx = static_cast<long long>(win.Mx); m.My = static_cast<long long>(win.My); m.W = static_cast<long long>(win.W);
+        m.Mxx = static_cast<long long>(win.Mxx); m.Myy = static_cast<long long>(win.Myy); m.Mxy = static_cast<long long>(win.Mxy);
+        m.N = N;
+        const float eig = eig_small_of(m, nullptr, nullptr, nullptr, nullptr);
+        wk.errs[o] = static_cast<float>(m.N) * eig;
+        if (++j == c_hi) break;
+        if (++o == cnt) o = 0;
+        if (++tr == cnt) tr = 0;
+        m6_add(win, m6_point(wk.keys[j]));
+        m6_sub(win, m6_point(wk.keys[tr]));
+      }
+    }
+  } else {
+#pragma unroll 1
+    for (uint32_t i = gt; i < cnt; i += GS) {
+      uint32_t i0 = i + cnt - ksz, i1 = i + ksz;
+      if (i0 >= cnt) i0 -= cnt;
+      if (i1 >= cnt) i1 -= cnt;
+      const Mom m = read_moments<MODE>(wk, cnt, i0, i1);
+      const float eig = eig_small_of(m, nullptr, nullptr, nullptr, nullptr);
+      wk.errs[i] = static_cast<float>(m.N) * eig;
+    }
   }
   gsync<GS>();
   if (KEEP && wk.errs != p.errs + pbase) {
@@ -849,35 +994,71 @@
 #pragma unroll 1
     for (uint32_t i = gt; i < cnt; i += GS) out[i] = wk.errs[i];
   }
-#pragma unroll 1
-  for (uint32_t i = gt; i < cnt; i += GS) {
+  if (MODE == kLfThreadSums && c_lo < c_hi) {
     const float kf[7] = {0.01110899634659290314f, 0.13533528149127960205f, 0.60653066635131835938f, 1.0f,
                          0.60653066635131835938f, 0.13533528149127960205f, 0.01110899634659290314f};
-    double acc = 0.0;
-    uint32_t q = i + cnt - 3;
+    float e[8];
+    uint32_t q = c_lo + cnt - 4;
     if (q >= cnt) q -= cnt;
 #pragma unroll
-    for (int j = 0; j < 7; j++) {
-      const double e = static_cast<double>(wk.errs[q]);
-      acc += e * static_cast<double>(kf[j]);
+    for (int j = 0; j < 8; j++) {
+      e[j] = wk.errs[q];
       if (++q == cnt) q = 0;
     }
-    wk.filt[i] = acc;
-  }
-  gsync<GS>();
-  if (KEEP && wk.filt != p.filt + pbase) {
-    double *out = p.filt + pbase;
+    double fm = 0.0, f0 = 0.0;
+#pragma unroll
+    for (int j = 0; j < 7; j++) fm += static_cast<double>(e[j]) * static_cast<double>(kf[j]);
+#pragma unroll
+    for (int j = 0; j < 7; j++) f0 += static_cast<double>(e[j + 1]) * static_cast<double>(kf[j]);
 #pragma unroll 1
-    for (uint32_t i = gt; i < cnt; i += GS) out[i] = wk.filt[i];
-  }
-
-#pragma unroll 1
-  for (uint32_t i = gt; i < cnt; i += GS) {
-    const double m = wk.filt[i];
-    const double bv = wk.filt[i == 0 ? cnt - 1 : i - 1], av = wk.filt[i + 1 == cnt ? 0 : i + 1];
-    if (m > bv && m > av) {
-      const uint32_t at = atomicAdd(&S.npeaks, 1u);
-      wk.peaks[at] = (static_cast<unsigned long long>(float_order(static_cast<float>(-m))) << 32) | i;
+    for (uint32_t i = c_lo; i < c_hi; i++) {
+#pragma unroll
+      for (int j = 0; j < 7; j++) e[j] = e[j + 1];
+      e[7] = wk.errs[q];
+      if (++q == cnt) q = 0;
+      double fp = 0.0;
+#pragma unroll
+      for (int j = 0; j < 7; j++) fp += static_cast<double>(e[j + 1]) * static_cast<double>(kf[j]);
+      if (KEEP) p.filt[pbase + i] = f0;
+      if (f0 > fm && f0 > fp) {
+        const uint32_t at = atomicAdd(&S.npeaks, 1u);
+        wk.peaks[at] = (static_cast<unsigned long long>(float_order(static_cast<float>(-f0))) << 32) | i;
+      }
+      fm = f0;
+      f0 = fp;
+    }
+  }
+  if constexpr (MODE != kLfThreadSums) {
+  #pragma unroll 1
+    for (uint32_t i = gt; i < cnt; i += GS) {
+      const float kf[7] = {0.01110899634659290314f, 0.13533528149127960205f, 0.60653066635131835938f, 1.0f,
+                           0.60653066635131835938f, 0.13533528149127960205f, 0.01110899634659290314f};
+      double acc = 0.0;
+      uint32_t q = i + cnt - 3;
+      if (q >= cnt) q -= cnt;
+  #pragma unroll
+      for (int j = 0; j < 7; j++) {
+        const double e = static_cast<double>(wk.errs[q]);
+        acc += e * static_cast<double>(kf[j]);
+        if (++q == cnt) q = 0;
+      }
+      wk.filt[i] = acc;
+    }
+    gsync<GS>();
+    if (KEEP && wk.filt != p.filt + pbase) {
+      double *out = p.filt + pbase;
+  #pragma unroll 1
+      for (uint32_t i = gt; i < cnt; i += GS) out[i] = wk.filt[i];
+    }
+
+  #pragma unroll 1
+    for (uint32_t i = gt; i < cnt; i += GS) {
+      const double m = wk.filt[i];
+      const double bv = wk.filt[i == 0 ? cnt - 1 : i - 1], av = wk.filt[i + 1 == cnt ? 0 : i + 1];
+      if (m > bv && m > av) {
+        const uint32_t at = atomicAdd(&S.npeaks, 1u);
+        wk.peaks[at] = (static_cast<unsigned long long>(float_order(static_cast<float>(-m))) << 32) | i;
+      }
     }
   }
   gsync<GS>();
@@ -934,15 +1115,23 @@
       PeakTable *t = p.peak_tables + static_cast<size_t>(frame) * p.blob_cap + fq;
       if (lane == 0) {
         t->blob = b; t->cnt = cnt; t->nsel = nm; t->npk = npk; t->rep0 = blob_rec->rep0; t->rep1 = blob_rec->rep1;
-        t->last = lf_load<AOS>(wk.lf, cnt - 1);
+        if constexpr (MODE != kLfThreadSums) t->last = lf_load<MODE>(wk, cnt - 1);
+        else t->last = m6_lfp(sums_at<GS>(wk.sums, GS - 1));
       }
       if (lane < static_cast<int>(nm)) {
         const uint32_t i = S.peak_idx[lane];
         t->idx[lane] = i;
-        t->at[lane] = lf_load<AOS>(wk.lf, i);
         b200tag_lfp z;
         z.Mxx = 0; z.Myy = 0; z.Mxy = 0; z.Mx = 0; z.My = 0; z.W = 0;
-        t->before[lane] = i > 0 ? lf_load<AOS>(wk.lf, i - 1) : z;
+        if constexpr (MODE != kLfThreadSums) {
+          t->at[lane] = lf_load<MODE>(wk, i);
+          t->before[lane] = i > 0 ? lf_load<MODE>(wk, i - 1) : z;
+        } else {
+          M6 before = i > 0 ? prefix_at<GS>(wk.keys, wk.sums, L, cnt, i - 1) : m6_zero();
+          t->before[lane] = m6_lfp(before);
+          m6_add(before, m6_point(wk.keys[i]));
+          t->at[lane] = m6_lfp(before);
+        }
       }
     }
   }
@@ -1140,11 +1329,37 @@
   }
 }
 
+__device__ __forceinline__ void carve_arrays(BlobWork &wk, unsigned char *base, uint32_t cap) {
+  wk.keys = reinterpret_cast<unsigned long long *>(base);
+  wk.m64 = reinterpret_cast<unsigned long long *>(base + 8ull * cap);
+  wk.m32 = reinterpret_cast<uint32_t *>(base + 32ull * cap);
+  wk.lf_cap = cap;
+  wk.errs = reinterpret_cast<float *>(base + 44ull * cap);
+  wk.lf = nullptr; wk.sums = nullptr;
+  wk.filt = reinterpret_cast<double *>(wk.keys);
+  wk.peaks = reinterpret_cast<unsigned long long *>(wk.errs);
+  wk.keys_in_place = false;
+  wk.hist = reinterpret_cast<uint32_t *>(wk.m64); wk.hist_cap = next_pow2(cap); wk.tmp = wk.hist + next_pow2(cap);
+}
+__host__ __device__ constexpr size_t smem_x_bytes(uint32_t cap, int threads) {
+  return (4ull * next_pow2(cap) + 4ull * cap) > (48ull * threads + 8ull * (cap / 2)) ? (4ull * next_pow2(cap) + 4ull * cap)
+                                                                                   : (48ull * threads + 8ull * (cap / 2));
+}
+__host__ __device__ constexpr size_t smem_blob_bytes(uint32_t cap, int threads) { return 12ull * cap + smem_x_bytes(cap, threads); }
+template <int GS>
+__device__ __forceinline__ void carve_smem(BlobWork &wk, unsigned char *base, uint32_t cap) {
+  wk.keys = reinterpret_cast<unsigned long long *>(base);
+  wk.errs = reinterpret_cast<float *>(base + 8ull * cap);
+  unsigned char *x = base + 12ull * cap;
+  wk.hist = reinterpret_cast<uint32_t *>(x); wk.hist_cap = next_pow2(cap); wk.tmp = wk.hist + next_pow2(cap);
+  wk.sums = reinterpret_cast<unsigned long long *>(x);
+  wk.peaks = wk.sums + 6 * GS;
+  wk.lf = nullptr; wk.m64 = nullptr; wk.m32 = nullptr; wk.lf_cap = 0; wk.filt = nullptr;
+  wk.keys_in_place = false;
+}
+
 struct SmallWarpShared {
-  unsigned long long keys[kSmallBlobPoints];
-  unsigned long long lf64[3 * kSmallBlobPoints];
-  uint32_t lf32[3 * kSmallBlobPoints];
-  alignas(16) float errs[kSmallBlobPoints];
+  alignas(16) unsigned char buf[48 * kSmallBlobPoints];
   BlobScratch<1> scratch;
 };
 
@@ -1159,15 +1374,7 @@
   const WorkItem *list = p.small_list + static_cast<size_t>(frame) * p.blob_cap;
   const uint32_t nlist = min(alloc_small(ctr->alloc), p.blob_cap);
   BlobWork wk;
-  wk.keys = S.keys;
-  wk.lf.aos = nullptr; wk.lf.m64 = S.lf64; wk.lf.m32 = S.lf32; wk.lf.cap = kSmallBlobPoints;
-  wk.errs = S.errs;
-  wk.filt = reinterpret_cast<double *>(S.keys);
-  wk.peaks = reinterpret_cast<unsigned long long *>(S.errs);
-  wk.keys_in_place = false;
-  wk.hist = reinterpret_cast<uint32_t *>(S.lf64);
-  wk.hist_cap = next_pow2(kSmallBlobPoints);
-  wk.tmp = wk.hist + next_pow2(kSmallBlobPoints);
+  carve_arrays(wk, S.buf, kSmallBlobPoints);
   uint32_t nxt = 0;
   if (lane == 0) nxt = atomicAdd(&ctr->next_small, 1u);
   while (true) {
@@ -1179,33 +1386,32 @@
     const uint32_t b = item.blob, off = item.offset, cnt = item.count;
     if (b >= p.blob_cap) continue;
     if (cnt > kSmallBlobPoints) continue;
-    fit_one_blob<32, false, KEEP>(p, frame, ctr, b, cnt, off, blobs + b, wk, S.scratch, nullptr, lane);
-  }
-}
-
-template <int THREADS, uint32_t KEY_CAP, uint32_t LF_CAP>
+    fit_one_blob<32, kLfArrays, KEEP>(p, frame, ctr, b, cnt, off, blobs + b, wk, S.scratch, nullptr, lane);
+  }
+}
+
+template <int THREADS, uint32_t CAP_A, uint32_t CAP_S, uint32_t KEY_CAP>
 struct CtaShared {
-  static constexpr bool kHasB = KEY_CAP > LF_CAP;
-  static constexpr uint32_t kScanWords = kHasB ? (KEY_CAP / 2 > 6 * THREADS ? KEY_CAP / 2 : 6 * THREADS) : 0;
-  static constexpr size_t kBytesA = static_cast<size_t>(LF_CAP) * 48;
-  static constexpr size_t kBytesB = kHasB ? static_cast<size_t>(KEY_CAP) * 12 + static_cast<size_t>(kScanWords) * 8 : 0;
-  alignas(16) unsigned char buf[kBytesA > kBytesB ? kBytesA : kBytesB];
+  static constexpr uint32_t kSmemCap = CAP_A > CAP_S ? CAP_A : CAP_S;
+  static constexpr bool kHasG = KEY_CAP > kSmemCap;
+  static constexpr uint32_t kScanWords = kHasG ? (KEY_CAP / 2 > 6 * THREADS ? KEY_CAP / 2 : 6 * THREADS) : 0;
+  static constexpr size_t kBytesA = 48ull * CAP_A;
+  static constexpr size_t kBytesS = CAP_S > 0 ? smem_blob_bytes(CAP_S, THREADS) : 0;
+  static constexpr size_t kBytesG = kHasG ? static_cast<size_t>(KEY_CAP) * 12 + static_cast<size_t>(kScanWords) * 8 : 0;
+  static constexpr size_t kBytesAS = kBytesA > kBytesS ? kBytesA : kBytesS;
+  alignas(16) unsigned char buf[kBytesAS > kBytesG ? kBytesAS : kBytesG];
   long long tot[6 * (THREADS / 32)];
   BlobScratch<THREADS / 32> scratch;
 
-  __device__ unsigned long long *a_keys() { return reinterpret_cast<unsigned long long *>(buf); }
-  __device__ unsigned long long *a_lf64() { return reinterpret_cast<unsigned long long *>(buf) + LF_CAP; }
-  __device__ uint32_t *a_lf32() { return reinterpret_cast<uint32_t *>(buf + static_cast<size_t>(LF_CAP) * 32); }
-  __device__ float *a_errs() { return reinterpret_cast<float *>(buf + static_cast<size_t>(LF_CAP) * 44); }
-  __device__ unsigned long long *b_keys() { return reinterpret_cast<unsigned long long *>(buf); }
-  __device__ float *b_errs() { return reinterpret_cast<float *>(buf + static_cast<size_t>(KEY_CAP) * 8); }
-  __device__ long long *b_scan() { return reinterpret_cast<long long *>(buf + static_cast<size_t>(KEY_CAP) * 12); }
+  __device__ unsigned long long *g_keys() { return reinterpret_cast<unsigned long long *>(buf); }
+  __device__ float *g_errs() { return reinterpret_cast<float *>(buf + static_cast<size_t>(KEY_CAP) * 8); }
+  __device__ unsigned long long *g_scan() { return reinterpret_cast<unsigned long long *>(buf + static_cast<size_t>(KEY_CAP) * 12); }
 };
-static_assert(kMediumCap % 4 == 0 && kSortCap % 4 == 0, "16-byte alignment of the carved arrays");
-
-template <int THREADS, uint32_t KEY_CAP, uint32_t LF_CAP, uint32_t MIN_CNT, uint32_t MAX_CNT, int MIN_CTAS, bool KEEP>
+
+template <int THREADS, uint32_t CAP_A, uint32_t CAP_S, uint32_t KEY_CAP, uint32_t MIN_CNT, uint32_t MAX_CNT, int MIN_CTAS, bool KEEP>
 __global__ void __launch_bounds__(THREADS, MIN_CTAS) k_fit_cta(FrameParams p, int tier) {
-  using Shared = CtaShared<THREADS, KEY_CAP, LF_CAP>;
+  using Shared = CtaShared<THREADS, CAP_A, CAP_S, KEY_CAP>;
+  static_assert(CAP_A % 4 == 0 && CAP_S % 4 == 0 && KEY_CAP % 4 == 0, "16-byte alignment of the carved arrays");
   extern __shared__ __align__(16) unsigned char smem_raw[];
   Shared &S = *reinterpret_cast<Shared *>(smem_raw);
   const int frame = blockIdx.y;
@@ -1231,52 +1437,61 @@
     if (blob_cnt < MIN_CNT || blob_cnt > MAX_CNT) continue;
     const size_t pbase = static_cast<size_t>(frame) * p.point_cap + blob_off;
     BlobWork wk;
-    constexpr bool kHasSmemLf = LF_CAP > 0;
-    constexpr bool kHasGlobalLf = MAX_CNT > LF_CAP;
+    constexpr bool kHasA = CAP_A > 0 && MIN_CNT <= CAP_A;
+    constexpr bool kHasS = CAP_S > CAP_A && MAX_CNT > CAP_A;
+    constexpr bool kHasG = Shared::kHasG && MAX_CNT > Shared::kSmemCap;
+    constexpr bool kGSums = kHasG && kHasS;
     constexpr bool kHasInPlace = MAX_CNT > KEY_CAP;
-    const bool lf32_ok = LF_CAP <= 1452 || !kHasGlobalLf ||
-                         static_cast<uint64_t>(blob_cnt) * 361u * (2u * static_cast<uint32_t>(max(p.w, p.h)) + 1u) < (1ull << 32);
-    if (kHasSmemLf && blob_cnt <= LF_CAP && lf32_ok) {
-      wk.keys = S.a_keys(); wk.errs = S.a_errs();
-      wk.lf.aos = nullptr; wk.lf.m64 = S.a_lf64(); wk.lf.m32 = S.a_lf32(); wk.lf.cap = LF_CAP;
-      wk.filt = reinterpret_cast<double *>(S.a_keys());
-      wk.peaks = reinterpret_cast<unsigned long long *>(S.a_errs());
+    const bool in_g = blob_cnt > Shared::kSmemCap && blob_cnt <= KEY_CAP;
+    if (kHasA && blob_cnt <= CAP_A) {
+      carve_arrays(wk, S.buf, CAP_A);
+      fit_one_blob<THREADS, kLfArrays, KEEP>(p, frame, ctr, b, blob_cnt, blob_off, blobs + b, wk, S.scratch, S.tot, tid);
+    } else if ((kHasS && blob_cnt <= CAP_S) || (kGSums && in_g)) {
+      if (kHasS && blob_cnt <= CAP_S) {
+        carve_smem<THREADS>(wk, S.buf, CAP_S);
+      } else {
+        wk.keys = S.g_keys(); wk.errs = S.g_errs();
+        wk.keys_in_place = false;
+        wk.hist = reinterpret_cast<uint32_t *>(S.g_scan()); wk.hist_cap = kScanHist; wk.tmp = reinterpret_cast<uint32_t *>(p.lfp + pbase);
+        wk.m64 = nullptr; wk.m32 = nullptr; wk.lf_cap = 0;
+        wk.lf = nullptr; wk.sums = S.g_scan(); wk.filt = nullptr;
+        wk.peaks = reinterpret_cast<unsigned long long *>(p.peak_ws + static_cast<size_t>(frame) * (p.point_cap / 2 + 1) + blob_off / 2);
+      }
+      fit_one_blob<THREADS, kLfThreadSums, KEEP>(p, frame, ctr, b, blob_cnt, blob_off, blobs + b, wk, S.scratch, S.tot, tid);
+    } else if (kHasG && !kGSums && in_g) {
+      wk.keys = S.g_keys(); wk.errs = S.g_errs();
       wk.keys_in_place = false;
-      wk.hist = reinterpret_cast<uint32_t *>(S.a_lf64()); wk.hist_cap = next_pow2(LF_CAP > 0 ? LF_CAP : 1); wk.tmp = wk.hist + next_pow2(LF_CAP > 0 ? LF_CAP : 1);
-      fit_one_blob<THREADS, false, KEEP>(p, frame, ctr, b, blob_cnt, blob_off, blobs + b, wk, S.scratch, S.tot, tid);
-    } else if (kHasGlobalLf && KEY_CAP > LF_CAP && blob_cnt <= KEY_CAP) {
-      wk.keys = S.b_keys(); wk.errs = S.b_errs();
-      wk.lf.aos = p.lfp + pbase; wk.lf.m64 = nullptr; wk.lf.m32 = nullptr; wk.lf.cap = 0;
-      wk.filt = reinterpret_cast<double *>(S.b_keys());
-      wk.peaks = reinterpret_cast<unsigned long long *>(S.b_errs());
-      wk.keys_in_place = false;
-      wk.hist = reinterpret_cast<uint32_t *>(S.b_scan()); wk.hist_cap = kScanHist; wk.tmp = reinterpret_cast<uint32_t *>(p.lfp + pbase);
-      fit_one_blob<THREADS, true, KEEP>(p, frame, ctr, b, blob_cnt, blob_off, blobs + b, wk, S.scratch, S.b_scan(), tid);
-    } else if (kHasInPlace) {
+      wk.hist = reinterpret_cast<uint32_t *>(S.g_scan()); wk.hist_cap = kScanHist; wk.tmp = reinterpret_cast<uint32_t *>(p.lfp + pbase);
+      wk.m64 = nullptr; wk.m32 = nullptr; wk.lf_cap = 0;
+      wk.lf = p.lfp + pbase; wk.sums = nullptr;
+      wk.filt = reinterpret_cast<double *>(S.g_keys()); wk.peaks = reinterpret_cast<unsigned long long *>(S.g_errs());
+      fit_one_blob<THREADS, kLfGlobal, KEEP>(p, frame, ctr, b, blob_cnt, blob_off, blobs + b, wk, S.scratch, reinterpret_cast<long long *>(S.g_scan()), tid);
+    } else if (kHasInPlace && blob_cnt > KEY_CAP) {
       wk.keys = reinterpret_cast<unsigned long long *>(p.seg_keys + pbase);
-      wk.lf.aos = p.lfp + pbase; wk.lf.m64 = nullptr; wk.lf.m32 = nullptr; wk.lf.cap = 0;
+      wk.lf = p.lfp + pbase; wk.sums = nullptr; wk.m64 = nullptr; wk.m32 = nullptr; wk.lf_cap = 0;
       wk.errs = p.errs + pbase; wk.filt = p.filt + pbase;
       wk.peaks = reinterpret_cast<unsigned long long *>(p.peak_ws + static_cast<size_t>(frame) * (p.point_cap / 2 + 1) + blob_off / 2);
       wk.keys_in_place = true;
-      wk.hist = reinterpret_cast<uint32_t *>(S.b_scan()); wk.hist_cap = kScanHist; wk.tmp = reinterpret_cast<uint32_t *>(p.lfp + pbase);
-      fit_one_blob<THREADS, true, KEEP>(p, frame, ctr, b, blob_cnt, blob_off, blobs + b, wk, S.scratch, S.b_scan(), tid);
-    }
-  }
-}
-
-using MediumShared = CtaShared<128, kMediumCap, kMediumCap>;
-constexpr uint32_t kLargeLfCap = 1536;
-using LargeShared = CtaShared<kLargeThreads, kSortCap, kLargeLfCap>;
+      wk.hist = reinterpret_cast<uint32_t *>(S.g_scan()); wk.hist_cap = kScanHist; wk.tmp = reinterpret_cast<uint32_t *>(p.lfp + pbase);
+      fit_one_blob<THREADS, kLfGlobal, KEEP>(p, frame, ctr, b, blob_cnt, blob_off, blobs + b, wk, S.scratch, reinterpret_cast<long long *>(S.g_scan()), tid);
+    }
+  }
+}
+
+using MediumShared = CtaShared<128, kMediumCap, 0, kMediumCap>;
+constexpr uint32_t kLargeArrCap = 1536;
+constexpr uint32_t kLargeSmemCap = 3648;
+using LargeShared = CtaShared<kLargeThreads, kLargeArrCap, kLargeSmemCap, kSortCap>;
 static_assert(sizeof(LargeShared) <= 76800 - 1024, "three CTAs of the large tier per SM");
 static_assert(sizeof(MediumShared) <= 37888, "shared memory of the medium tier");
-#define K_FIT_MEDIUM(KEEP) k_fit_cta<128, kMediumCap, kMediumCap, kSmallBlobPoints + 1, kMediumCap, 6, KEEP>
-#define K_FIT_LARGE(KEEP) k_fit_cta<kLargeThreads, kSortCap, kLargeLfCap, kMediumCap + 1, kSortCap, 3, KEEP>
+#define K_FIT_MEDIUM(KEEP) k_fit_cta<128, kMediumCap, 0, kMediumCap, kSmallBlobPoints + 1, kMediumCap, 6, KEEP>
+#define K_FIT_LARGE(KEEP) k_fit_cta<kLargeThreads, kLargeArrCap, kLargeSmemCap, kSortCap, kMediumCap + 1, kSortCap, (KEEP) ? 2 : 3, KEEP>
 constexpr int kHugeThreads = 512;
 constexpr uint32_t kHugeCap = 8192;
-using HugeShared = CtaShared<kHugeThreads, kHugeCap, 0>;
-#define K_FIT_HUGE(KEEP) k_fit_cta<kHugeThreads, kHugeCap, 0, kSortCap + 1, 0xffffffffu, (KEEP) ? 1 : 2, KEEP>
-using Large512Shared = CtaShared<kHugeThreads, kSortCap, kSortCap>;
-#define K_FIT_LARGE512(KEEP) k_fit_cta<kHugeThreads, kSortCap, kSortCap, kMediumCap + 1, kSortCap, 1, KEEP>
+using HugeShared = CtaShared<kHugeThreads, 0, 0, kHugeCap>;
+#define K_FIT_HUGE(KEEP) k_fit_cta<kHugeThreads, 0, 0, kHugeCap, kSortCap + 1, 0xffffffffu, (KEEP) ? 1 : 2, KEEP>
+using Large512Shared = CtaShared<kHugeThreads, kSortCap, 0, kSortCap>;
+#define K_FIT_LARGE512(KEEP) k_fit_cta<kHugeThreads, kSortCap, 0, kSortCap, kMediumCap + 1, kSortCap, 1, KEEP>
 static_assert(sizeof(Large512Shared) <= 227 * 1024, "shared memory of the low-latency large tier");
 constexpr int kLowLatencyFrames = 4;
 
```

After: 60140, median of 6. 2.5% higher.
